# borgor/ripcurrents

Measured on AMD Instinct MI355X. Metric: frames/sec dense Farneback flow @1080p, higher is better.
Workload: dtype f32

## Files before the change

ripcurrents_amd/csrc/flow_iter_kernels.hip:

```cpp

#include <cstdlib>

#include "rc_device.h"

#define RC_ITER_BATCH 3
#define RC_RR_D 3

#ifdef RC_EXACT_BUILD
#define RC_FLOW_NS rc_flow_exact
#else
#define RC_FLOW_NS rc_flow_fast
#endif
namespace RC_FLOW_NS {

__device__ __forceinline__ float2 rc_flow_in(const RcIterArgs& a, const float2* fin, int gx, int gy) {
    if (a.in_mode == 0) return make_float2(0.f, 0.f);
    if (a.in_mode == 1) return fin[(size_t)gy * a.w + gx];
    float ax, ay;
    int sx = rc_src_x(gx, a.up_scale_x, a.fin_w, ax);
    int sx1 = min(sx + 1, a.fin_w - 1);
    int sy = rc_src_y(gy, a.up_scale_y, ay);
    int sy0 = rc_clampi(sy, 0, a.fin_h - 1), sy1 = rc_clampi(sy + 1, 0, a.fin_h - 1);
    const float2* S0 = fin + (size_t)sy0 * a.fin_w;
    const float2* S1 = fin + (size_t)sy1 * a.fin_w;
// ... 447 lines not shown
    for (int idx = tid; idx < 5 * CH * (TW / 4); idx += NT) {
        const int g4 = idx % (TW / 4), row = (idx / (TW / 4)) % CH, c = idx / (CH * (TW / 4));
        const float4* vp = (const float4*)(V + c * CH * VP + row * VP + 4 * g4);
        float v[4 * NQ];
#pragma unroll
        for (int q = 0; q < NQ; q++) {
            float4 t = vp[q];
            v[4 * q] = t.x; v[4 * q + 1] = t.y; v[4 * q + 2] = t.z; v[4 * q + 3] = t.w;
        }
        float o[4];
#pragma unroll
        for (int p = 0; p < 4; p++) {
            float s = v[M_ + p] * a.win.k[0];
#pragma unroll
            for (int i = 1; i <= M_; i++) s += a.win.k[i] * (v[M_ + p - i] + v[M_ + p + i]);
            o[p] = s;
        }
        *(float4*)(G + c * RING * MP + row * TW + 4 * g4) = make_float4(o[0], o[1], o[2], o[3]);
    }
    __syncthreads();
    for (int px = tid; px < CH * TW; px += NT) {
        const int row = px / TW, lx = px - row * TW;
        const int gx = tx0 + lx, gy = Y + row;
        double g[5];
#pragma unroll
        for (int c = 0; c < 5; c++) g[c] = G[c * RING * MP + px];
        if (gx < a.w && gy < yend) *(float2*)(fout + (size_t)gy * a.fout_step + (size_t)gx * 8) = rc_solve(g);
    }
    __syncthreads();
}

template <int M_, int NT, int BATCH>
__global__ __launch_bounds__(NT) void k_flow_iter_sweep(RcIterArgs a) {
    using S = RcSweep<M_>;
    constexpr int CH = S::CH, MW = S::MW, MP = S::MP, RING = S::RING, TW = S::TW;
    extern __shared__ __align__(16) float smf[];
    float* ring = smf;
    float* V = smf + 5 * RING * MP;
    const int tid = threadIdx.x;
    const int z = blockIdx.y;
    const int strip = blockIdx.x % a.tiles_x, seg = blockIdx.x / a.tiles_x;
    const int tx0 = strip * TW, y0 = seg * a.th;
    const int w = a.w, h = a.h;
    const int yend = min(y0 + a.th, h);
    const size_t s0 = (size_t)((a.slot0 + z * a.zstep) % a.nslots) * a.R_slot_stride;
    const size_t s1 = (size_t)((a.slot1 + z * a.zstep) % a.nslots) * a.R_slot_stride;
    const float4* RA0 = a.RA + s0;  const float* RB0 = a.RB + s0;
    const float4* RA1 = a.RA + s1;  const float* RB1 = a.RB + s1;
    const float2* fin = a.fin ? a.fin + (size_t)z * a.fin_pair_stride : nullptr;
    char* fout = a.fout + (size_t)z * a.fout_pair_stride;

    auto matrices_rows = [&](int r0, int nrows) {
        const int n = nrows * MW;
        for (int base = tid; base < n; base += NT * BATCH) {
            float2 d[BATCH];
            int gxs[BATCH], gys[BATCH];
#pragma unroll
            for (int q = 0; q < BATCH; q++) {
                const int idx = min(base + q * NT, n - 1);
                const int j = idx / MW, lx = idx - j * MW;
                gxs[q] = rc_clampi(tx0 - M_ + lx, 0, w - 1);
                gys[q] = rc_clampi(r0 + j, 0, h - 1);
                d[q] = rc_flow_in(a, fin, gxs[q], gys[q]);
            }
            RcM5 v[BATCH];
#pragma unroll
            for (int q = 0; q < BATCH; q++)
                v[q] = rc_matrices(RA0, RB0, RA1, RB1, gxs[q], gys[q], w, h, d[q].x, d[q].y);
#pragma unroll
            for (int q = 0; q < BATCH; q++) {
                const int idx = base + q * NT;
                if (idx < n) {
                    const int j = idx / MW, lx = idx - j * MW;
                    const int slot = (r0 + j - (y0 - M_)) % RING;
                    float* mp = ring + slot * MP + lx;
                    mp[0] = v[q].m0;
                    mp[RING * MP] = v[q].m1;
                    mp[2 * RING * MP] = v[q].m2;
                    mp[3 * RING * MP] = v[q].m3;
                    mp[4 * RING * MP] = v[q].m4;
                }
            }
        }
    };
    matrices_rows(y0 - M_, 2 * M_);
    const int nsteps = (yend - y0 + CH - 1) / CH;
    for (int s = 0; s < nsteps; s++) {
        matrices_rows(y0 + M_ + CH * s, CH);
        __syncthreads();
        const int Y = y0 + CH * s;
        switch (s % (RING / CH)) {
            case 0: rc_sweep_bc<M_, NT, 0>(a, ring, V, tid, tx0, Y, yend, fout); break;
            case 1: rc_sweep_bc<M_, NT, CH>(a, ring, V, tid, tx0, Y, yend, fout); break;
            case 2: rc_sweep_bc<M_, NT, 2 * CH>(a, ring, V, tid, tx0, Y, yend, fout); break;
            default: if constexpr (RING / CH > 3) rc_sweep_bc<M_, NT, 3 * CH>(a, ring, V, tid, tx0, Y, yend, fout); break;
        }
    }
}

template <int M, int NT, int BATCH>
static void launch_iter_sweep(RcIterArgs a, int pairs, hipStream_t s) {
    using S = RcSweep<M>;
    static_assert(S::RING / S::CH <= 4, "step dispatch covers four ring phases");
    RC_ALLOW_LDS((k_flow_iter_sweep<M, NT, BATCH>), S::LDS);
    a.tw = S::TW;
    a.tiles_x = (a.w + S::TW - 1) / S::TW;
    const int want = 4 * 512;
    int segs = (want + a.tiles_x * pairs - 1) / (a.tiles_x * pairs);
    int rs = (a.h + segs - 1) / segs;
    rs = ((rs + S::CH - 1) / S::CH) * S::CH;
    if (rs < 32) rs = 32;
    a.th = rs;
    a.tiles_y = (a.h + rs - 1) / rs;
    hipLaunchKernelGGL((k_flow_iter_sweep<M, NT, BATCH>), dim3(a.tiles_x * a.tiles_y, pairs, 1), dim3(NT), S::LDS, s, a);
}

#define RC_W3_THREADS 512
template <int IN_MODE, int GAUSS_>
__global__ __launch_bounds__(RC_W3_THREADS) void k_flow_iter_w3(RcIterArgs a) {
    constexpr int TW = 64, TH = 16, MW = TW + 2, MH = TH + 2, MP = MW | 1;
    constexpr int NITEMS = MW * MH, NIT = (NITEMS + RC_W3_THREADS - 1) / RC_W3_THREADS;
    extern __shared__ __align__(16) float smf[];
    float* Ms = smf;
    const int tid = threadIdx.x;
    const int z = blockIdx.y;
    const int t = a.xcd_remap ? rc_xcd_remap(blockIdx.x, a.tiles_x * a.tiles_y) : (int)blockIdx.x;
    const int tx0 = (t % a.tiles_x) * TW, ty0 = (t / a.tiles_x) * TH;
    const int w = a.w, h = a.h;
    const size_t s0 = (size_t)((a.slot0 + z * a.zstep) % a.nslots) * a.R_slot_stride;
    const size_t s1 = (size_t)((a.slot1 + z * a.zstep) % a.nslots) * a.R_slot_stride;
    const float4* __restrict__ RA0 = a.RA + s0;  const float* __restrict__ RB0 = a.RB + s0;
    const float4* __restrict__ RA1 = a.RA + s1;  const float* __restrict__ RB1 = a.RB + s1;
    const float2* __restrict__ fin = a.fin + (size_t)z * a.fin_pair_stride;
    char* fout = a.fout + (size_t)z * a.fout_pair_stride;

    int gx[NIT], gy[NIT];
#pragma unroll
    for (int q = 0; q < NIT; q++) {
        int idx = min(tid + q * RC_W3_THREADS, NITEMS - 1);
        int ly = idx / MW, lx = idx - ly * MW;
        gx[q] = rc_clampi(tx0 - 1 + lx, 0, w - 1);
        gy[q] = rc_clampi(ty0 - 1 + ly, 0, h - 1);
    }
    float dx[NIT], dy[NIT];
    if constexpr (IN_MODE == 0) {
#pragma unroll
        for (int q = 0; q < NIT; q++) dx[q] = dy[q] = 0.f;
    } else if constexpr (IN_MODE == 1) {
        float2 d[NIT];
#pragma unroll
        for (int q = 0; q < NIT; q++) d[q] = fin[(size_t)gy[q] * w + gx[q]];
#pragma unroll
        for (int q = 0; q < NIT; q++) { dx[q] = d[q].x; dy[q] = d[q].y; }
    } else {
        float2 p00[NIT], p01[NIT], p10[NIT], p11[NIT];
        float ax[NIT], ay[NIT];
#pragma unroll
        for (int q = 0; q < NIT; q++) {
            int sx = rc_src_x(gx[q], a.up_scale_x, a.fin_w, ax[q]);
            int sx1 = min(sx + 1, a.fin_w - 1);
            int sy = rc_src_y(gy[q], a.up_scale_y, ay[q]);
            int sy0 = rc_clampi(sy, 0, a.fin_h - 1), sy1 = rc_clampi(sy + 1, 0, a.fin_h - 1);
            const float2* S0 = fin + (size_t)sy0 * a.fin_w;
            const float2* S1 = fin + (size_t)sy1 * a.fin_w;
            p00[q] = S0[sx]; p01[q] = S0[sx1]; p10[q] = S1[sx]; p11[q] = S1[sx1];
        }
#pragma unroll
        for (int q = 0; q < NIT; q++) {
            float a0 = 1.f - ax[q], a1 = ax[q], b0 = 1.f - ay[q], b1 = ay[q];
            float r0x = p00[q].x * a0 + p01[q].x * a1, r1x = p10[q].x * a0 + p11[q].x * a1;
            float r0y = p00[q].y * a0 + p01[q].y * a1, r1y = p10[q].y * a0 + p11[q].y * a1;
            dx[q] = (r0x * b0 + r1x * b1) * a.up_mul;
            dy[q] = (r0y * b0 + r1y * b1) * a.up_mul;
        }
    }
    float4 A0[NIT];
    float B0[NIT];
    RcGather gt[NIT];
#pragma unroll
    for (int q = 0; q < NIT; q++) {
        size_t p0 = (size_t)gy[q] * w + gx[q];
        A0[q] = RA0[p0];
        B0[q] = RB0[p0];
        rc_gather_issue(gt[q], RA1, RB1, gx[q], gy[q], dx[q], dy[q], w, h);
    }
#pragma unroll
    for (int q = 0; q < NIT; q++) {
        RcM5 v = rc_matrices_reg(A0[q], B0[q], gt[q], dx[q], dy[q], gx[q], gy[q], w, h);
        int idx = tid + q * RC_W3_THREADS;
        if (idx < NITEMS) {
            int ly = idx / MW, lx = idx - ly * MW;
            float* mp = Ms + ly * MP + lx;
            mp[0] = v.m0;
            mp[MH * MP] = v.m1;
            mp[2 * MH * MP] = v.m2;
            mp[3 * MH * MP] = v.m3;
            mp[4 * MH * MP] = v.m4;
        }
    }
    __syncthreads();

    constexpr int RPT = TH / (RC_W3_THREADS / TW);
    const int lx = tid % TW, r0 = (tid / TW) * RPT;
    const int ox = tx0 + lx;
    float g[RPT][5];
#pragma unroll
    for (int c = 0; c < 5; c++) {
        const float* mc = Ms + c * MH * MP + r0 * MP + lx;
        float col[3][RPT + 2];
#pragma unroll
        for (int j = 0; j < 3; j++)
#pragma unroll
            for (int r = 0; r < RPT + 2; r++) col[j][r] = mc[r * MP + j];
#pragma unroll
        for (int r = 0; r < RPT; r++) {
            float v[3];
#pragma unroll
            for (int j = 0; j < 3; j++) {
                if (GAUSS_) v[j] = col[j][r + 1] * a.win.k[0] + (col[j][r + 2] + col[j][r]) * a.win.k[1];
                else v[j] = col[j][r + 1] + (col[j][r + 2] + col[j][r]);
            }
            if (GAUSS_) g[r][c] = v[1] * a.win.k[0] + a.win.k[1] * (v[0] + v[2]);
            else g[r][c] = (v[1] + v[0]) + v[2];
        }
    }
    if (ox < w) {
#pragma unroll
        for (int r = 0; r < RPT; r++) {
            int oy = ty0 + r0 + r;
            if (oy < h)
                *(float2*)(fout + (size_t)oy * a.fout_step + (size_t)ox * 8) =
                    rc_solve3(g[r], GAUSS_ ? 1e-3f : (float)a.win.box_eps);
        }
    }
}

template <int IN_MODE, int G>
static void launch_w3(RcIterArgs a, int pairs, hipStream_t s) {
    a.tw = 64; a.th = 16;
    a.tiles_x = (a.w + 63) / 64; a.tiles_y = (a.h + 15) / 16;
    size_t lds = sizeof(float) * 5 * 18 * 67;
    hipLaunchKernelGGL((k_flow_iter_w3<IN_MODE, G>), dim3(a.tiles_x * a.tiles_y, pairs, 1), dim3(RC_W3_THREADS), lds, s, a);
}

template <int WW, int WH, int WP = WW>
__device__ __forceinline__ void rc_gather_window(RcGather& g, const float4* LA, const float* LB, int ox, int oy,
                                                 const float4* __restrict__ RA1, const float* __restrict__ RB1,
                                                 int gx, int gy, float dx, float dy, int w, int h) {
    float fx = gx + dx, fy = gy + dy;
    int x1 = (int)floorf(fx), y1 = (int)floorf(fy);
    g.fx = fx - x1;
    g.fy = fy - y1;
    g.inside = (unsigned)x1 < (unsigned)(w - 1) && (unsigned)y1 < (unsigned)(h - 1);
    const int wx = x1 - ox, wy = y1 - oy;
    if (g.inside && (unsigned)wx < (unsigned)(WW - 1) && (unsigned)wy < (unsigned)(WH - 1)) {
        const int i = wy * WP + wx;
        g.q00 = LA[i]; g.q01 = LA[i + 1]; g.q10 = LA[i + WP]; g.q11 = LA[i + WP + 1];
        g.e00 = LB[i]; g.e01 = LB[i + 1]; g.e10 = LB[i + WP]; g.e11 = LB[i + WP + 1];
    } else {
        const size_t p = g.inside ? (size_t)y1 * w + x1 : (size_t)gy * w + gx;
        const size_t pw = g.inside ? (size_t)w : 0, p1 = g.inside ? 1 : 0;
        g.q00 = RA1[p]; g.q01 = RA1[p + p1]; g.q10 = RA1[p + pw]; g.q11 = RA1[p + pw + p1];
        g.e00 = RB1[p]; g.e01 = RB1[p + p1]; g.e10 = RB1[p + pw]; g.e11 = RB1[p + pw + p1];
    }
}

__device__ __forceinline__ void rc_hsum3_dpp(float (&g)[5], const float (&V)[5]) {
    float t0, t1, t2, t3, t4;
    asm("s_nop 1\n\t"
        "v_add_f32_dpp %5, %10, %10 wave_shr:1 row_mask:0xf bank_mask:0xf bound_ctrl:1\n\t"
        "v_add_f32_dpp %6, %11, %11 wave_shr:1 row_mask:0xf bank_mask:0xf bound_ctrl:1\n\t"
        "v_add_f32_dpp %7, %12, %12 wave_shr:1 row_mask:0xf bank_mask:0xf bound_ctrl:1\n\t"
        "v_add_f32_dpp %8, %13, %13 wave_shr:1 row_mask:0xf bank_mask:0xf bound_ctrl:1\n\t"
        "v_add_f32_dpp %9, %14, %14 wave_shr:1 row_mask:0xf bank_mask:0xf bound_ctrl:1\n\t"
        "v_add_f32_dpp %0, %10, %5 wave_shl:1 row_mask:0xf bank_mask:0xf bound_ctrl:1\n\t"
        "v_add_f32_dpp %1, %11, %6 wave_shl:1 row_mask:0xf bank_mask:0xf bound_ctrl:1\n\t"
        "v_add_f32_dpp %2, %12, %7 wave_shl:1 row_mask:0xf bank_mask:0xf bound_ctrl:1\n\t"
        "v_add_f32_dpp %3, %13, %8 wave_shl:1 row_mask:0xf bank_mask:0xf bound_ctrl:1\n\t"
        "v_add_f32_dpp %4, %14, %9 wave_shl:1 row_mask:0xf bank_mask:0xf bound_ctrl:1"
        : "=&v"(g[0]), "=&v"(g[1]), "=&v"(g[2]), "=&v"(g[3]), "=&v"(g[4]),
          "=&v"(t0), "=&v"(t1), "=&v"(t2), "=&v"(t3), "=&v"(t4)
        : "v"(V[0]), "v"(V[1]), "v"(V[2]), "v"(V[3]), "v"(V[4]));
}


__device__ __forceinline__ void rc_hpair_dpp(float (&s)[5], const float (&V)[5]) {
    float t0, t1, t2, t3, t4;
    asm("s_nop 1\n\t"
        "v_mov_b32_dpp %5, %10 wave_shr:1 row_mask:0xf bank_mask:0xf bound_ctrl:1\n\t"
        "v_mov_b32_dpp %6, %11 wave_shr:1 row_mask:0xf bank_mask:0xf bound_ctrl:1\n\t"
        "v_mov_b32_dpp %7, %12 wave_shr:1 row_mask:0xf bank_mask:0xf bound_ctrl:1\n\t"
        "v_mov_b32_dpp %8, %13 wave_shr:1 row_mask:0xf bank_mask:0xf bound_ctrl:1\n\t"
        "v_mov_b32_dpp %9, %14 wave_shr:1 row_mask:0xf bank_mask:0xf bound_ctrl:1\n\t"
        "v_add_f32_dpp %0, %10, %5 wave_shl:1 row_mask:0xf bank_mask:0xf bound_ctrl:1\n\t"
        "v_add_f32_dpp %1, %11, %6 wave_shl:1 row_mask:0xf bank_mask:0xf bound_ctrl:1\n\t"
        "v_add_f32_dpp %2, %12, %7 wave_shl:1 row_mask:0xf bank_mask:0xf bound_ctrl:1\n\t"
        "v_add_f32_dpp %3, %13, %8 wave_shl:1 row_mask:0xf bank_mask:0xf bound_ctrl:1\n\t"
        "v_add_f32_dpp %4, %14, %9 wave_shl:1 row_mask:0xf bank_mask:0xf bound_ctrl:1"
        : "=&v"(s[0]), "=&v"(s[1]), "=&v"(s[2]), "=&v"(s[3]), "=&v"(s[4]),
          "=&v"(t0), "=&v"(t1), "=&v"(t2), "=&v"(t3), "=&v"(t4)
        : "v"(V[0]), "v"(V[1]), "v"(V[2]), "v"(V[3]), "v"(V[4]));
}

template <int GAUSS_, int NIT, int MW, int NG>
__device__ __forceinline__ void rc_rr_flows(const float (&m)[NIT][5], const float* XR, int grp, int x,
                                            const RcWindow& win, float2 (&f)[NIT]) {
    const int gu = max(grp - 1, 0), gd = min(grp + 1, NG - 1);
    const int bu = (int)__umul24((unsigned)gu, 10u * MW) + x, bd = (int)__umul24((unsigned)gd, 10u * MW) + x;
    float up[5], dn[5];
#pragma unroll
    for (int c = 0; c < 5; c++) {
        up[c] = XR[bu + (5 + c) * MW];
        dn[c] = XR[bd + c * MW];
    }
    float V[NIT][5];
#pragma unroll
    for (int q = 0; q < NIT; q++)
#pragma unroll
        for (int c = 0; c < 5; c++) {
            float u = q > 0 ? m[q - 1][c] : up[c], d = q < NIT - 1 ? m[q + 1][c] : dn[c];
            if (GAUSS_) V[q][c] = m[q][c] * win.k[0] + (d + u) * win.k[1];
            else V[q][c] = m[q][c] + (d + u);
        }
#pragma unroll
    for (int q = 0; q < NIT; q++) {
        float g[5];
        if (GAUSS_) {
            float lr[5];
            rc_hpair_dpp(lr, V[q]);
#pragma unroll
            for (int c = 0; c < 5; c++) g[c] = V[q][c] * win.k[0] + win.k[1] * lr[c];
        } else {
            rc_hsum3_dpp(g, V[q]);
        }
        f[q] = rc_solve3(g, GAUSS_ ? 1e-3f : (float)win.box_eps);
    }
}

template <int NIT, int MW>
__device__ __forceinline__ void rc_rr_exchange(const float (&m)[NIT][5], float* XR, int grp, int x) {
    const int b = (int)__umul24((unsigned)grp, 10u * MW) + x;
#pragma unroll
    for (int c = 0; c < 5; c++) {
        XR[b + c * MW] = m[0][c];
        XR[b + (5 + c) * MW] = m[NIT - 1][c];
    }
}

template <int IN_MODE, int NIT, int MW, int MH, bool INTERIOR = false>
__device__ __forceinline__ void rc_rr_flow_in(const RcIterArgs& a, const float2* __restrict__ fin, int tx0, int ty0,
                                              int gxo, const int (&gys)[NIT], float (&dx)[NIT], float (&dy)[NIT]) {
    const int w = a.w, h = a.h;
    if constexpr (IN_MODE == 0) {
#pragma unroll
        for (int q = 0; q < NIT; q++) dx[q] = dy[q] = 0.f;
    } else if constexpr (IN_MODE == 1) {
        float2 d[NIT];
#pragma unroll
        for (int q = 0; q < NIT; q++) d[q] = INTERIOR ? fin[(unsigned)(gys[q] * w + gxo)] : fin[(size_t)gys[q] * w + gxo];
#pragma unroll
        for (int q = 0; q < NIT; q++) { dx[q] = d[q].x; dy[q] = d[q].y; }
    } else if ((NIT % 2 == 0) && a.up_exact2 && (INTERIOR || (ty0 - 2 >= 0 && ty0 - 2 + MH <= h))) {
        constexpr int NR = NIT / 2 + 2;
        int sx = (gxo - 1) >> 1;
        float ax = (gxo & 1) ? 0.25f : 0.75f;
        if (!INTERIOR) {
            if (sx < 0) { ax = 0.f; sx = 0; }
            if (sx >= a.fin_w - 1) { ax = 0.f; sx = a.fin_w - 1; }
        }
        const int sx1 = min(sx + 1, a.fin_w - 1);
        const int rb = (gys[0] - 1) >> 1;
        float2 t0[NR], t1[NR];
        typedef float rc_f4a8 __attribute__((ext_vector_type(4), aligned(8)));
        const bool cols_plain = INTERIOR || (tx0 - 2 >= 1 && tx0 - 2 + MW <= w && ((tx0 - 2 + MW - 2) >> 1) + 1 <= a.fin_w - 1);
        if (INTERIOR) {
            unsigned co = (unsigned)(__mul24(rb, a.fin_w) + sx);
#pragma unroll
            for (int j = 0; j < NR; j++) {
                const rc_f4a8 v = *(const rc_f4a8*)(fin + co);
                t0[j] = make_float2(v.x, v.y); t1[j] = make_float2(v.z, v.w);
                co += (unsigned)a.fin_w;
            }
        } else if (cols_plain) {
#pragma unroll
            for (int j = 0; j < NR; j++) {
                const float2* S = fin + (size_t)rc_clampi(rb + j, 0, a.fin_h - 1) * a.fin_w;
                const rc_f4a8 v = *(const rc_f4a8*)(S + sx);
                t0[j] = make_float2(v.x, v.y); t1[j] = make_float2(v.z, v.w);
            }
        } else {
#pragma unroll
            for (int j = 0; j < NR; j++) {
                const float2* S = fin + (size_t)rc_clampi(rb + j, 0, a.fin_h - 1) * a.fin_w;
                t0[j] = S[sx]; t1[j] = S[sx1];
            }
        }
        const float a0 = 1.f - ax, a1 = ax;
        float hx[NR], hy[NR];
#pragma unroll
        for (int j = 0; j < NR; j++) {
            hx[j] = t0[j].x * a0 + t1[j].x * a1;
            hy[j] = t0[j].y * a0 + t1[j].y * a1;
        }
#pragma unroll
        for (int q = 0; q < NIT; q++) {
            const int j0 = (q + 1) >> 1;
            const float b1 = (q & 1) ? 0.25f : 0.75f, b0 = 1.f - b1;
            dx[q] = (hx[j0] * b0 + hx[j0 + 1] * b1) * a.up_mul;
            dy[q] = (hy[j0] * b0 + hy[j0 + 1] * b1) * a.up_mul;
        }
    } else {
        float2 p00[NIT], p01[NIT], p10[NIT], p11[NIT];
        float ax, ay[NIT];
        int sx, sys[NIT];
        if (a.up_exact2) {
            sx = (gxo - 1) >> 1;
            ax = (gxo & 1) ? 0.25f : 0.75f;
            if (sx < 0) { ax = 0.f; sx = 0; }
            if (sx >= a.fin_w - 1) { ax = 0.f; sx = a.fin_w - 1; }
#pragma unroll
            for (int q = 0; q < NIT; q++) { sys[q] = (gys[q] - 1) >> 1; ay[q] = (gys[q] & 1) ? 0.25f : 0.75f; }
        } else {
            sx = rc_src_x(gxo, a.up_scale_x, a.fin_w, ax);
#pragma unroll
            for (int q = 0; q < NIT; q++) sys[q] = rc_src_y(gys[q], a.up_scale_y, ay[q]);
        }
        const int sx1 = min(sx + 1, a.fin_w - 1);
#pragma unroll
        for (int q = 0; q < NIT; q++) {
            int sy = sys[q];
            int sy0 = rc_clampi(sy, 0, a.fin_h - 1), sy1 = rc_clampi(sy + 1, 0, a.fin_h - 1);
            const float2* S0 = fin + (size_t)sy0 * a.fin_w;
            const float2* S1 = fin + (size_t)sy1 * a.fin_w;
            p00[q] = S0[sx]; p01[q] = S0[sx1]; p10[q] = S1[sx]; p11[q] = S1[sx1];
        }
#pragma unroll
        for (int q = 0; q < NIT; q++) {
            float a0 = 1.f - ax, a1 = ax, b0 = 1.f - ay[q], b1 = ay[q];
            float r0x = p00[q].x * a0 + p01[q].x * a1, r1x = p10[q].x * a0 + p11[q].x * a1;
            float r0y = p00[q].y * a0 + p01[q].y * a1, r1y = p10[q].y * a0 + p11[q].y * a1;
            dx[q] = (r0x * b0 + r1x * b1) * a.up_mul;
            dy[q] = (r0y * b0 + r1y * b1) * a.up_mul;
        }
    }
}


__device__ __forceinline__ void rc_lds_barrier() { asm volatile("s_waitcnt lgkmcnt(0)\n\ts_barrier" ::: "memory"); }
__device__ __forceinline__ void rc_all_barrier() { asm volatile("s_waitcnt vmcnt(0) lgkmcnt(0)\n\ts_barrier" ::: "memory"); }

constexpr bool rc_recip_exact(int nt, int wp) {
    const unsigned r = (65536u + wp - 1) / wp;
    for (int t = 0; t < nt; t++)
        if ((int)((t * r) >> 16) != t / wp) return false;
    return true;
}

__device__ __forceinline__ void rc_glds16_s(const void* base, unsigned voff, uint32_t lds_wave_addr) {
    asm volatile("s_mov_b32 m0, %2\n\ts_nop 0\n\tglobal_load_lds_dwordx4 %0, %1" ::"v"(voff), "s"(base), "s"(lds_wave_addr) : "memory");
}
__device__ __forceinline__ void rc_glds4_s(const void* base, unsigned voff, uint32_t lds_wave_addr) {
    asm volatile("s_mov_b32 m0, %2\n\ts_nop 0\n\tglobal_load_lds_dword %0, %1" ::"v"(voff), "s"(base), "s"(lds_wave_addr) : "memory");
}

template <bool INTERIOR, int NT, int WP, int WN, int NWL>
__device__ __forceinline__ void rc_rrc_issue_window(const float4* __restrict__ RA1, const float* __restrict__ RB1,
                                                    uint32_t lds_a, uint32_t lds_b, int tid, int ox, int oy, int w, int h) {
    constexpr int QY = NT / WP, QX = NT % WP;
    const int wave_base = __builtin_amdgcn_readfirstlane(tid & ~63);
    static_assert(rc_recip_exact(NT, WP), "tid / WP by multiply and shift must be exact for every thread");
    int wy = (int)(__umul24((unsigned)tid, (65536u + WP - 1) / WP) >> 16), wx = tid - (int)__umul24((unsigned)wy, (unsigned)WP);
    int off = __mul24(oy + wy, w) + ox + wx;
#pragma unroll
    for (int q = 0; q < NWL; q++) {
        bool ok = (q + 1) * NT <= WN || tid + q * NT < WN;
        if (!INTERIOR) ok = ok && (unsigned)(ox + wx) < (unsigned)w && (unsigned)(oy + wy) < (unsigned)h;
        const unsigned p = ok ? (unsigned)off : 0u;
        if (q * NT + wave_base < WN) {
            rc_glds16_s(RA1, p << 4, lds_a + (uint32_t)(q * NT + wave_base) * 16u);
            rc_glds4_s(RB1, p << 2, lds_b + (uint32_t)(q * NT + wave_base) * 4u);
        }
        wx += QX; wy += QY; off += QY * w + QX;
        if (wx >= WP) { wx -= WP; wy += 1; off += w - WP; }
    }
}

template <bool INTERIOR, int NIT, int WW, int WH, int WP>
__device__ __forceinline__ void rc_rr_matrices(float (&m)[NIT][5], const float4 (&A0)[NIT], const float (&B0)[NIT],
                                               const float (&dx)[NIT], const float (&dy)[NIT], const float4* LA,
                                               const float* LB, int ox, int oy, const float4* __restrict__ RA1,
                                               const float* __restrict__ RB1, int gxo, const int (&gys)[NIT], int w, int h) {
    if constexpr (!INTERIOR) {
#pragma unroll
        for (int q = 0; q < NIT; q++) {
            RcGather g;
            rc_gather_window<WW, WH, WP>(g, LA, LB, ox, oy, RA1, RB1, gxo, gys[q], dx[q], dy[q], w, h);
            RcM5 v = rc_matrices_reg(A0[q], B0[q], g, dx[q], dy[q], gxo, gys[q], w, h, true);
            m[q][0] = v.m0; m[q][1] = v.m1; m[q][2] = v.m2; m[q][3] = v.m3; m[q][4] = v.m4;
        }
    } else {
        unsigned far = 0;
#pragma unroll
        for (int q = 0; q < NIT; q++) {
            RcGather g;
            const float fx = gxo + dx[q], fy = gys[q] + dy[q];
            const float flx = floorf(fx), fly = floorf(fy);
            const int x1 = (int)flx, y1 = (int)fly;
            g.fx = fx - flx;
            g.fy = fy - fly;
            g.inside = true;
            const int wx = x1 - ox, wy = y1 - oy;
            const bool in_win = (unsigned)wx < (unsigned)(WW - 1) && (unsigned)wy < (unsigned)(WH - 1);
            far |= in_win ? 0u : 1u << q;
            const unsigned i = in_win ? __umul24((unsigned)wy, (unsigned)WP) + (unsigned)wx : 0u;
            const float4* pa = (const float4*)((const char*)LA + (i << 4));
            const float* pb = (const float*)((const char*)LB + (i << 2));
            g.q00 = pa[0]; g.q01 = pa[1]; g.q10 = pa[WP]; g.q11 = pa[WP + 1];
            g.e00 = pb[0]; g.e01 = pb[1]; g.e10 = pb[WP]; g.e11 = pb[WP + 1];
            RcM5 v = rc_matrices_reg(A0[q], B0[q], g, dx[q], dy[q], gxo, gys[q], w, h, false);
            m[q][0] = v.m0; m[q][1] = v.m1; m[q][2] = v.m2; m[q][3] = v.m3; m[q][4] = v.m4;
        }
        if (__builtin_expect(far != 0, 0)) {
#pragma unroll
            for (int q = 0; q < NIT; q++) {
                if (far >> q & 1) {
                    RcGather g;
                    rc_gather_issue(g, RA1, RB1, gxo, gys[q], dx[q], dy[q], w, h);
                    RcM5 v = rc_matrices_reg(A0[q], B0[q], g, dx[q], dy[q], gxo, gys[q], w, h, false);
                    m[q][0] = v.m0; m[q][1] = v.m1; m[q][2] = v.m2; m[q][3] = v.m3; m[q][4] = v.m4;
                }
            }
        }
    }
}

template <bool INTERIOR, int IN_MODE, int GAUSS_, int NIT, int D, int MW, int NG>
__device__ __forceinline__ void rc_rrc_body(const RcIterArgs& a, const int zb, const int ze, float* smf, const uint32_t lds0, const int tx0, const int ty0) {
    constexpr int NT = NG * MW, MH = NG * NIT;
    constexpr int WW = MW + 2 * D, WH = MH + 2 * D, WP = WW, WN = WP * WH, NWL = (WN + NT - 1) / NT;
    constexpr int WNP = (WN + 63) & ~63;
    constexpr int MP = MW + 1, PLANE = MH * MP;
    static_assert(5 * PLANE <= 5 * WNP, "border-block M1 planes alias the R1 window");
    float4* LA = (float4*)smf;
    float* LB = smf + 4 * WNP;
    float* XR = LB + WNP;
    float* Ms = smf;
    const uint32_t lds_a = lds0, lds_b = lds0 + 16u * WNP;
    const int w = a.w, h = a.h;
    const int ox = tx0 - 2 - D, oy = ty0 - 2 - D;
#define RC_RRC_COORDS(tid_)                                                         \
    const int x = (tid_) & (MW - 1), grp = (tid_) / MW, ly0 = grp * NIT;            \
    const int px = tx0 - 2 + x;                                                     \
    const int gxo = INTERIOR ? px : rc_clampi(px, 0, w - 1);                        \
    int gys[NIT];                                                                   \
    _Pragma("unroll") for (int q = 0; q < NIT; q++)                                 \
        gys[q] = INTERIOR ? ty0 - 2 + ly0 + q : rc_clampi(ty0 - 2 + ly0 + q, 0, h - 1);

    float4 A0[NIT];
    float B0[NIT];
    float dx[NIT], dy[NIT];
    {
        const int tid = threadIdx.x;
        RC_RRC_COORDS(tid)
        const size_t s0 = (size_t)((a.slot0 + zb * a.zstep) % a.nslots) * a.R_slot_stride;
        const size_t s1 = (size_t)((a.slot1 + zb * a.zstep) % a.nslots) * a.R_slot_stride;
        rc_rrc_issue_window<INTERIOR, NT, WP, WN, NWL>(a.RA + s1, a.RB + s1, lds_a, lds_b, tid, ox, oy, w, h);
#pragma unroll
        for (int q = 0; q < NIT; q++) {
            const unsigned p0 = (unsigned)(gys[q] * w + gxo);
            A0[q] = (a.RA + s0)[p0];
            B0[q] = (a.RB + s0)[p0];
        }
        rc_rr_flow_in<IN_MODE, NIT, MW, MH, INTERIOR>(a, a.fin + (size_t)zb * a.fin_pair_stride, tx0, ty0, gxo, gys, dx, dy);
    }

    for (int z = zb; z < ze; z++) {
        const size_t s1 = (size_t)((a.slot1 + z * a.zstep) % a.nslots) * a.R_slot_stride;
        const float4* __restrict__ RA1 = a.RA + s1;
        const float* __restrict__ RB1 = a.RB + s1;
        const bool more = z + 1 < ze;
        int tid = threadIdx.x;
        asm volatile("" : "+v"(tid));
        RC_RRC_COORDS(tid)
        rc_all_barrier();

        float m[NIT][5];
        rc_rr_matrices<INTERIOR, NIT, WW, WH, WP>(m, A0, B0, dx, dy, LA, LB, ox, oy, RA1, RB1, gxo, gys, w, h);
        rc_rr_exchange<NIT, MW>(m, XR, grp, x);
        rc_lds_barrier();

        {
            float2 f1[NIT];
            rc_rr_flows<GAUSS_, NIT, MW, NG>(m, XR, grp, x, a.win, f1);
            float f1x[NIT], f1y[NIT];
#pragma unroll
            for (int q = 0; q < NIT; q++) { f1x[q] = f1[q].x; f1y[q] = f1[q].y; }
            rc_rr_matrices<INTERIOR, NIT, WW, WH, WP>(m, A0, B0, f1x, f1y, LA, LB, ox, oy, RA1, RB1, gxo, gys, w, h);
        }
        if (more) {
#pragma unroll
            for (int q = 0; q < NIT; q++) {
                const int i = (int)__umul24((unsigned)(gys[q] - oy), (unsigned)WP) + (gxo - ox);
                A0[q] = LA[i];
                B0[q] = LB[i];
            }
        }
        rc_lds_barrier();
        if constexpr (!INTERIOR) {
#pragma unroll
            for (int q = 0; q < NIT; q++)
#pragma unroll
                for (int c = 0; c < 5; c++) Ms[c * PLANE + (ly0 + q) * MP + x] = m[q][c];
            rc_lds_barrier();
#pragma unroll
            for (int q = 0; q < NIT; q++) {
                const int py = ty0 - 2 + ly0 + q;
                if ((unsigned)px >= (unsigned)w || (unsigned)py >= (unsigned)h) {
                    const int cx = gxo - (tx0 - 2), cy = gys[q] - (ty0 - 2);
#pragma unroll
                    for (int c = 0; c < 5; c++) m[q][c] = Ms[c * PLANE + cy * MP + cx];
                }
            }
        }
        rc_rr_exchange<NIT, MW>(m, XR, grp, x);
        rc_lds_barrier();

        if (more) {
            const size_t n1 = (size_t)((a.slot1 + (z + 1) * a.zstep) % a.nslots) * a.R_slot_stride;
            rc_rrc_issue_window<INTERIOR, NT, WP, WN, NWL>(a.RA + n1, a.RB + n1, lds_a, lds_b, tid, ox, oy, w, h);
        }

        {
            char* fout = a.fout + (size_t)z * a.fout_pair_stride;
            float2 f2[NIT];
            rc_rr_flows<GAUSS_, NIT, MW, NG>(m, XR, grp, x, a.win, f2);
            if (x >= 2 && x < MW - 2 && (INTERIOR || px < w)) {
                unsigned so = (unsigned)(ty0 - 2 + ly0) * (unsigned)a.fout_step + (unsigned)px * 8u;
#pragma unroll
                for (int q = 0; q < NIT; q++) {
                    const int ly = ly0 + q, py = ty0 - 2 + ly;
                    if (ly >= 2 && ly < MH - 2 && (INTERIOR || py < h)) *(float2*)(fout + so) = f2[q];
                    so += (unsigned)a.fout_step;
                }
            }
        }
        if (more) rc_rr_flow_in<IN_MODE, NIT, MW, MH, INTERIOR>(a, a.fin + (size_t)(z + 1) * a.fin_pair_stride, tx0, ty0, gxo, gys, dx, dy);
    }
#undef RC_RRC_COORDS
}

template <int IN_MODE, int GAUSS_, int NIT, int D, int MINB, int MW, int NG>
__global__ __launch_bounds__(NG * MW, MINB) void k_flow_iter2_rrc(RcIterArgs a, RcChainPlan cp) {
    constexpr int MH = NG * NIT, TW = MW - 4, TH = MH - 4;
    extern __shared__ __align__(16) float smf[];
    const int zb = cp.ngroups ? cp.start[blockIdx.y] : (int)blockIdx.y, ze = cp.ngroups ? cp.start[blockIdx.y + 1] : zb + 1;
    const int t = a.xcd_remap ? rc_xcd_remap(blockIdx.x, a.tiles_x * a.tiles_y) : (int)blockIdx.x;
    const int tx0 = (t % a.tiles_x) * TW, ty0 = (t / a.tiles_x) * TH;
    const bool interior = tx0 - 2 >= 5 && tx0 - 2 + MW <= a.w - 5 && ty0 - 2 >= 5 && ty0 - 2 + MH <= a.h - 5;
    const uint32_t lds0 = (uint32_t)(uintptr_t)(__attribute__((address_space(3))) void*)smf;
    if (interior) rc_rrc_body<true, IN_MODE, GAUSS_, NIT, D, MW, NG>(a, zb, ze, smf, lds0, tx0, ty0);
    else rc_rrc_body<false, IN_MODE, GAUSS_, NIT, D, MW, NG>(a, zb, ze, smf, lds0, tx0, ty0);
}

template <int IN_MODE, int G, int NIT, int D, int MINB, int MW = 32, int NG = 8>
static void launch_rrc_t(RcIterArgs a, const RcChainPlan& cp, int pairs, hipStream_t s) {
    constexpr int MH = NG * NIT, TW = MW - 4, TH = MH - 4;
    a.tw = TW; a.th = TH;
    a.tiles_x = (a.w + TW - 1) / TW; a.tiles_y = (a.h + TH - 1) / TH;
    constexpr int WN = (MW + 2 * D) * (MH + 2 * D), WNP = (WN + 63) & ~63;
    const size_t lds = sizeof(float) * (5 * WNP + NG * 2 * 5 * MW);
    RC_ALLOW_LDS((k_flow_iter2_rrc<IN_MODE, G, NIT, D, MINB, MW, NG>), lds);
    hipLaunchKernelGGL((k_flow_iter2_rrc<IN_MODE, G, NIT, D, MINB, MW, NG>), dim3(a.tiles_x * a.tiles_y, cp.ngroups ? cp.ngroups : pairs, 1), dim3(NG * MW), lds, s, a, cp);
}

static void rc_chain_plan(const RcIterArgs& a, int pairs, long long tiles, RcChainPlan& cp) {
    cp.ngroups = 0;
    const bool chainable = a.chain > 1 && pairs > 1 && (a.slot0 + a.zstep) % a.nslots == a.slot1 % a.nslots;
    if (!chainable) return;
    int chain = a.chain;
    if (!(a.ablate & RC_ABL_FORCE_CHAIN))
        while (chain > 1 && tiles * pairs / chain < (a.chain_min_blocks > 0 ? a.chain_min_blocks : 4096)) chain >>= 1;
    if (chain <= 1) return;
    int n = 0, z = 0;
    cp.start[0] = 0;
    while (z < pairs) {
        int left = pairs - z, c = left > chain ? chain : (left + 1) / 2;
        if (n == RC_MAX_CHAIN_GROUPS - 1) c = left;
        z += c;
        cp.start[++n] = z;
    }
    cp.ngroups = n;
}

template <int IN_MODE, int G>
static void launch_w3x2(RcIterArgs a, int pairs, hipStream_t s) {
    const long long tiles = (long long)((a.w + 27) / 28) * ((a.h + 27) / 28), blocks = tiles * pairs;
    RcChainPlan cp;
    rc_chain_plan(a, pairs, tiles, cp);
    if (cp.ngroups) launch_rrc_t<IN_MODE, G, 4, RC_RR_D, 4>(a, cp, pairs, s);
    else if (blocks < 512) launch_rrc_t<IN_MODE, G, 2, 4, 6>(a, cp, pairs, s);
    else if (blocks < 1024) launch_rrc_t<IN_MODE, G, 3, 4, 5>(a, cp, pairs, s);
    else launch_rrc_t<IN_MODE, G, 4, RC_RR_D, 4>(a, cp, pairs, s);
}

int rc_flow_iter_can_fuse2(const RcIterArgs& a) { return a.win.m == 1 && a.solve && a.addr32; }

int rc_flow_iter2_r0_reads(const RcIterArgs& a, int pairs) {
    RcChainPlan cp;
    rc_chain_plan(a, pairs, (long long)((a.w + 27) / 28) * ((a.h + 27) / 28), cp);
    return cp.ngroups ? cp.ngroups : pairs;
}

int rc_flow_chain_groups(const RcIterArgs& a, int pairs, int* starts, int cap) {
    RcChainPlan cp;
    rc_chain_plan(a, pairs, (long long)((a.w + 27) / 28) * ((a.h + 27) / 28), cp);
    for (int i = 0; i <= cp.ngroups && i < cap; i++) starts[i] = cp.start[i];
    return cp.ngroups;
}

void rc_launch_flow_iter2(const RcIterArgs& a, int pairs, hipStream_t s) {
    const int g = a.win.gaussian ? 1 : 0;
    switch (a.in_mode * 2 + g) {
        case 0: launch_w3x2<0, 0>(a, pairs, s); break;
        case 1: launch_w3x2<0, 1>(a, pairs, s); break;
        case 2: launch_w3x2<1, 0>(a, pairs, s); break;
        case 3: launch_w3x2<1, 1>(a, pairs, s); break;
        case 4: launch_w3x2<2, 0>(a, pairs, s); break;
        default: launch_w3x2<2, 1>(a, pairs, s); break;
    }
}

static size_t iter_lds(int tw, int th, int m, bool two_buffers) {
    int MW = tw + 2 * m, MH = th + 2 * m, MP = MW | 1;
    return sizeof(float) * (5 * (size_t)MH * MP + (two_buffers ? 5 * (size_t)th * MP : 0));
}

template <int TW, int TH, int M, int G>
static void launch_iter_t(RcIterArgs a, int pairs, hipStream_t s) {
    size_t lds = iter_lds(TW, TH, M, M > 1);
    RC_ALLOW_LDS((k_flow_iter<TW, TH, M, G>), lds);
    a.tw = TW; a.th = TH;
    a.tiles_x = (a.w + TW - 1) / TW; a.tiles_y = (a.h + TH - 1) / TH;
    hipLaunchKernelGGL((k_flow_iter<TW, TH, M, G>), dim3(a.tiles_x * a.tiles_y, pairs, 1), dim3(RC_BLOCK), lds, s, a);
}

static void pick_runtime_tile(int m, int& tw, int& th) {
    static const int tiles[][2] = {{64, 16}, {32, 32}, {64, 8}, {32, 16}, {16, 16}, {16, 8}, {8, 8}};
    double best = -1;
    tw = 8; th = 8;
    for (auto& t : tiles) {
        size_t lds = iter_lds(t[0], t[1], m, true);
        if (lds > 150 * 1024) continue;
        double eff = (double)(t[0] * t[1]) / ((t[0] + 2 * m) * (t[1] + 2 * m));
        if (lds > 64 * 1024) eff *= 0.6;
        if (t[0] < 64) eff *= 0.95;
        if (eff > best) { best = eff; tw = t[0]; th = t[1]; }
    }
}

void rc_launch_flow_iter(const RcIterArgs& a, int pairs, hipStream_t s) {
    const int m = a.win.m, g = a.win.gaussian ? 1 : 0;
    if (m == 1 && a.solve) {
        switch (a.in_mode * 2 + g) {
            case 0: launch_w3<0, 0>(a, pairs, s); break;
            case 1: launch_w3<0, 1>(a, pairs, s); break;
            case 2: launch_w3<1, 0>(a, pairs, s); break;
            case 3: launch_w3<1, 1>(a, pairs, s); break;
            case 4: launch_w3<2, 0>(a, pairs, s); break;
            default: launch_w3<2, 1>(a, pairs, s); break;
        }
        return;
    }
    if (m == 1) { g ? launch_iter_t<64, 16, 1, 1>(a, pairs, s) : launch_iter_t<64, 16, 1, 0>(a, pairs, s); return; }
    if (a.solve) {
        if (m == 2) { g ? launch_iter_big<2, 1, 512>(a, pairs, s) : launch_iter_big<2, 0, 512>(a, pairs, s); return; }
        const long long work = (long long)a.w * a.h * pairs;
        if (g && (m == 5 || m == 10) && !(a.ablate & RC_ABL_TILE_WINDOW) &&
            ((a.ablate & RC_ABL_FORCE_SWEEP) || work >= (m == 10 ? 900000ll : 8000000ll))) {
            m == 5 ? launch_iter_sweep<5, 1024, 1>(a, pairs, s) : launch_iter_sweep<10, 1024, 1>(a, pairs, s);
            return;
        }
        if (m == 5) { g ? launch_iter_big<5, 1, 1024>(a, pairs, s) : launch_iter_big<5, 0, 1024>(a, pairs, s); return; }
        if (m == 10) { g ? launch_iter_big<10, 1, 1024, 64>(a, pairs, s) : launch_iter_big<10, 0, 1024, 64>(a, pairs, s); return; }
    }
    if (m == 2) { g ? launch_iter_t<64, 16, 2, 1>(a, pairs, s) : launch_iter_t<64, 16, 2, 0>(a, pairs, s); return; }
    if (m == 5) { g ? launch_iter_t<32, 32, 5, 1>(a, pairs, s) : launch_iter_t<32, 32, 5, 0>(a, pairs, s); return; }
    if (m == 10) { g ? launch_iter_t<32, 32, 10, 1>(a, pairs, s) : launch_iter_t<32, 32, 10, 0>(a, pairs, s); return; }
    RcIterArgs b = a;
    pick_runtime_tile(m, b.tw, b.th);
    b.tiles_x = (b.w + b.tw - 1) / b.tw; b.tiles_y = (b.h + b.th - 1) / b.th;
    size_t lds = iter_lds(b.tw, b.th, m, true);
    RC_ALLOW_LDS((k_flow_iter<0, 0, 0, 0>), lds);
    hipLaunchKernelGGL((k_flow_iter<0, 0, 0, 0>), dim3(b.tiles_x * b.tiles_y, pairs, 1), dim3(RC_BLOCK), lds, s, b);
}

}
```

ripcurrents_amd/csrc/rc_common.h:

```cpp
#pragma once

#include <hip/hip_runtime.h>
#include <limits.h>
#include <stdint.h>

#include "../../include/rcflow.h"
#include "rc_plan.h"

#define RC_FMA(a, b, c) __builtin_fmaf((a), (b), (c))

__device__ __forceinline__ int rc_cvt_i32_x86(float v) {
    return (v >= -2147483648.f && v < 2147483648.f) ? (int)v : (int)0x80000000;
}

__device__ __forceinline__ const float2* rc_row2(const float* base, size_t step, int y) {
    return (const float2*)((const char*)base + (size_t)y * step);
}

__device__ __forceinline__ bool rc_sample_flow(const float* flow, size_t step, int w, int h, float x, float y,
                                               float& dx, float& dy) {
    int xind = rc_cvt_i32_x86(floorf(x)), yind = rc_cvt_i32_x86(floorf(y));
    float xrem = x - xind, yrem = y - yind;
    if (xind < 1 || yind < 1 || xind + 2 > w || yind + 2 > h) return false;
    const float2* r0 = rc_row2(flow, step, yind) + xind;
    const float2* r1 = rc_row2(flow, step, yind + 1) + xind;
    float2 p00 = r0[0], p01 = r0[1], p10 = r1[0], p11 = r1[1];
    float wa = 1 - xrem, wb = 1 - yrem;
    dx = p00.x * wa * wb + p01.x * xrem * wb + p10.x * wa * yrem + p11.x * xrem * yrem;
    dy = p00.y * wa * wb + p01.y * xrem * wb + p10.y * wa * yrem + p11.y * xrem * yrem;
    return true;
}

__device__ __forceinline__ uint8_t rc_f2u8(float v) {
    int iv;
    if (!(v > -2147483904.f && v < 2147483648.f)) iv = INT_MIN;
    else iv = (int)v;
    return (uint8_t)(iv & 0xFF);
}

struct RcPyrArgs {
    const uint8_t* src;
    size_t src_step;
    size_t src_frame_stride;
    int W0, H0;
    float* dst;
    size_t dst_slot_stride;
    int dslot0, nslots, zstep;
    int w, h;
    double scale_x, scale_y;
    int ksize;
    const float* kern;
    int tw, th, reg_wp, reg_hmax;
    int direct;
    int fixed3;
};

struct RcPyrFused {
    float* dst;
    size_t dst_slot_stride;
    int w, h;
    const float* kern;
};

struct RcPolyArgs {
    const float* I;
    size_t I_slot_stride;
    const uint8_t* src8;
    size_t src8_step, src8_frame_stride;
    float4* RA;
    float* RB;
    size_t R_slot_stride;
    int slot0, nslots, zstep;
    int w, h;
    int tile_h;
    int valu_vertical;
    RcPolyK pk;
    int npyr;
    RcPyrFused py[2];
};

enum RcAblate : int {
    RC_ABL_EXACT_PLAIN_SCANS = 2,
    RC_ABL_EXACT_FUSED_M = 16,
    RC_ABL_PYR_STAGED = 4096,
    RC_ABL_TILE_WINDOW = 65536,
    RC_ABL_FORCE_SWEEP = 8388608,
    RC_ABL_FORCE_CHAIN = 33554432,
};

struct RcIterArgs {
    const float4* RA;
    const float* RB;
    size_t R_slot_stride;
    int slot0, slot1, nslots, zstep;
    int w, h;
    int in_mode;
    const float2* fin;
    size_t fin_pair_stride;
    int fin_w, fin_h;
    double up_scale_x, up_scale_y;
    float up_mul;
    int up_exact2;
    char* fout;
    size_t fout_step;
    size_t fout_pair_stride;
    int tw, th;
    int tiles_x, tiles_y;
    int solve;
    int xcd_remap;
    int ablate;
    int addr32;
    int chain_min_blocks;
    int chain;
    RcWindow win;
};

#define RC_MAX_CHAIN_GROUPS 64
struct RcChainPlan {
    int ngroups;
    int start[RC_MAX_CHAIN_GROUPS + 1];
};

struct RcExactArgs {
    const float4* RA;
    const float* RB;
    size_t n;
    int slot0, slot1, nslots, zstep;
    int w, h;
    const float2* fin;
    size_t fin_pair_stride;
    int fin_w, fin_h;
    double up_scale_x, up_scale_y;
    float up_mul;
    float2* flow;
    float* M;
    void* V;
    void* G;
    char* out;
    size_t out_step, out_pair_stride;
    int plain_scans;
    int fused_matrices;
    RcWindow win;
};
void rc_launch_exact_polyexp(const RcPolyArgs& a, int frames, hipStream_t s);
void rc_launch_exact_flow_init(const RcExactArgs& a, int pairs, hipStream_t s);
void rc_launch_exact_matrices(const RcExactArgs& a, int pairs, hipStream_t s);
void rc_launch_exact_window_solve(const RcExactArgs& a, int pairs, hipStream_t s);
int rc_exact_iteration_fused_ok(const RcExactArgs& a);
void rc_launch_exact_iteration_fused(const RcExactArgs& a, int pairs, hipStream_t s);

#define RC_MAX_DEVICES 64
#define RC_ALLOW_LDS(fn, lds)                                                                             \
    do {                                                                                                  \
        static size_t rc_seen_[RC_MAX_DEVICES] = {0};                                                     \
        int rc_dev_ = 0;                                                                                  \
        (void)hipGetDevice(&rc_dev_);                                                                     \
        if (rc_dev_ >= 0 && rc_dev_ < RC_MAX_DEVICES && (size_t)(lds) > rc_seen_[rc_dev_]) {             \
            (void)hipFuncSetAttribute((const void*)(fn), hipFuncAttributeMaxDynamicSharedMemorySize, (int)(lds)); \
            rc_seen_[rc_dev_] = (size_t)(lds);                                                            \
        }                                                                                                 \
    } while (0)

void rc_launch_pyr(const RcPyrArgs& a, int frames, size_t lds, hipStream_t s);
void rc_launch_polyexp(const RcPolyArgs& a, int frames, hipStream_t s);
int rc_polyexp_pyr_ok(const RcPolyArgs& a);
int rc_pyr_pair_ok(const RcPyrArgs& a1, const RcPyrArgs& a2);
void rc_launch_pyr_pair(const RcPyrArgs& a1, const RcPyrArgs& a2, int frames, hipStream_t s);
int rc_polyexp_multi_ok(const RcPolyArgs* a, int nlev);
void rc_launch_polyexp_multi(const RcPolyArgs* a, int nlev, int frames, hipStream_t s);
#define RC_FLOW_DECLS                                                         \
    void rc_launch_flow_iter(const RcIterArgs& a, int pairs, hipStream_t s);  \
     \
    int rc_flow_iter_can_fuse2(const RcIterArgs& a);                          \
    int rc_flow_iter2_r0_reads(const RcIterArgs& a, int pairs);               \
    int rc_flow_chain_groups(const RcIterArgs& a, int pairs, int* starts, int cap); \
    void rc_launch_flow_iter2(const RcIterArgs& a, int pairs, hipStream_t s);
namespace rc_flow_fast { RC_FLOW_DECLS }
namespace rc_flow_exact { RC_FLOW_DECLS }

struct RcFlowAreaArgs {
    const char* src;
    size_t src_step;
    size_t src_pair_stride;
    int W, H;
    float2* dst;
    size_t dst_pair_stride;
    int w, h;
    float mul;
    int fast, ix, iy;
    const int* xstart; const int* xsi; const float* xalpha;
    const int* ystart; const int* ysi; const float* yalpha;
    int lds_tab;
};
void rc_launch_flow_area_init(const RcFlowAreaArgs& a, int pairs, hipStream_t s);

void rc_launch_pack_R5(const float* R5, float4* RA, float* RB, int n, int fast_scale, hipStream_t s);
void rc_launch_unpack_R5(const float4* RA, const float* RB, float* R5, int n, int fast_scale, hipStream_t s);
```

ripcurrents_amd/csrc/rc_host.h:

```cpp
#pragma once

#include <initializer_list>
#include <string>
#include <vector>

#include "rc_args.h"
#include "rc_common.h"

struct RcBuf {
    void* p = nullptr;
    size_t bytes = 0;
};

struct RcPlan {
    bool valid = false;
    int w = 0, h = 0;
    rc_farneback_params prm{};
    int nlev = 0;
    RcLevel lv[RC_MAX_LEVELS];
    size_t kern_off[RC_MAX_LEVELS];
    RcPolyK pk;
    RcWindow win;
    int nslots = 0, chunk = 0;
    int exact_taps = 0;
// ... 9 lines not shown
    RcBuf thr;
    RcBuf acc;
    RcBuf pt;
    RcBuf dist;
    RcBuf scratch;
    RcBuf jet;
    RcBuf loopc;
};

struct RcLkPyr {
    int top; bool deriv;
    int lw[8], lh[8];
    size_t offI[8], offD[8], bytes;
};

struct RcZeroFence {
    hipEvent_t ev = nullptr;
    hipStream_t stream = nullptr;
    bool pending = false;
};

struct RcTimex {
    bool open = false;
    int w = 0, h = 0, window = 0, products = 0;
    int pitch = 0;
    size_t plane = 0;
    int cur = 0;
    long long frames = 0;
    RcBuf sum;
    RcBuf ring;
    RcBuf avg;
    RcBuf bd_idx[2], bd_hsv[2];
    RcZeroFence zf;
};

struct RcFrameStab {
    bool open = false;
    int w = 0, h = 0;
    int rx = 0, ry = 0, rw = 0, rh = 0;
    int N = 0, M = 0;
    size_t lds = 0;
    long long frames = 0;
    RcBuf tab;
    RcBuf prev;
    RcBuf res;
    RcBuf scratch;
    RcZeroFence zf;
    int n = 0, model = 0, flags = 0;
    double min_response = 0.;
    int px[RC_STAB_MAX_PATCHES] = {}, py[RC_STAB_MAX_PATCHES] = {};
    bool tracks = false;
    rc_stab_tracks tp{};
    int ncells = 0, margin = 0;
    RcLkPyr ref{}, cur{};
    RcBuf lkref, lkcur;
    RcBuf trk;
    int pcur = 0; bool pflip = false;
};
enum { RC_FT_RESULT = 0 , RC_FT_FIT = 4 , RC_FT_WS = 16 , RC_FT_DOUBLES = 18 };
enum { RC_FS_RESULT = 0 , RC_FS_MOTION = 3 , RC_FS_USED = 9 ,
       RC_FS_TICKET = 10 , RC_FS_SHIFTS = 16  };

struct RcRipMap {
    bool open = false;
    int w = 0, h = 0, window = 0, gx = 0, gy = 0, source = 0, flags = 0;
    int pitch = 0;
    int cur = 0;
    long long frames = 0;
    double K = 0.3454915028125263;
    double M = 0.;
    RcBuf ring;
    RcBuf avg;
    RcBuf acc;
    RcBuf out;
    RcZeroFence zf;
};

struct RcTrLineH { int kind, cap, n0; long long t_add; };
struct RcTracers {
    bool open = false;
    int w = 0, h = 0;
    rc_tracers_params prm{};
    std::vector<RcTrLineH> lines;
    int reserved = 0;
    int init_n = 0;
    int cur = 0;
    long long t = 0, t_reset = 0;
    long long dropped = 0;
    bool primed = false; int pyr_cur = 0;
    int nprims = 0;
    RcLkPyr plan{};
    RcBuf pyr;
    RcBuf pos;
    RcBuf init;
    RcBuf tab;
    RcBuf prims;
    RcBuf status;
    RcBuf ctr;
    RcZeroFence zf;
};

struct RcRegions {
    bool open = false;
    int w = 0, h = 0;
    rc_regions_params prm{};
    long long pushes = 0;
    RcBuf par;
    RcBuf area;
    RcBuf rows;
    RcBuf acc;
    RcBuf out;
    RcZeroFence zf;
};

struct RcTracks {
    bool open = false;
    int w = 0, h = 0;
    rc_tracks_params prm{};
    long long pushes = 0;
    RcBuf foot;
    RcBuf ov;
    RcBuf aux;
    RcBuf out;
    RcZeroFence zf;
};

struct RcMotion {
    bool open = false;
    int w = 0, h = 0;
    rc_motion_params prm{};
    int pitch = 0;
    long long pushes = 0;
    double last_ts = 0.;
    RcBuf mhi;
    RcBuf prev;
    RcBuf orient;
    RcBuf mask;
    RcBuf tab;
    RcBuf out;
    RcZeroFence zf;
};

struct RcFtle {
    bool open = false;
    int w = 0, h = 0;
    rc_ftle_params prm{};
    int pitch = 0;
    int cur = 0;
    long long pushes = 0;
    RcBuf ring;
    RcBuf map;
    RcBuf steps;
    RcBuf lam;
    RcBuf ctl;
    RcBuf out;
    RcBuf jet;
    RcZeroFence zf;
};

struct RcPlanView {
    bool open = false;
    int w = 0, h = 0;
    rc_planview_params prm{};
    long long pushes = 0;
    RcBuf table;
    RcBuf ctl;
    RcBuf out;
    RcZeroFence zf;
};

struct RcWaves {
    bool open = false;
    int w = 0, h = 0;
    rc_waves_params prm{};
    int K = 0;
    int pitch = 0;
    int sh = 0;
    long long pushes = 0;
    std::vector<int> tc, ts;
    RcBuf ring;
    RcBuf acc;
    RcBuf cacc;
    RcBuf out;
    RcBuf jet;
    RcZeroFence zf;
};

struct RcPiv {
    bool open = false;
    int w = 0, h = 0;
    rc_piv_params prm{};
    int gx = 0, gy = 0;
    int nw = 0;
    int pitch = 0;
    long long pushes = 0;
    RcBuf prev;
    RcBuf ring;
    RcBuf acc;
    RcBuf out;
    RcBuf ctl;
    RcBuf jet;
    RcZeroFence zf;
};

struct RcTransects {
    bool open = false;
    int w = 0, h = 0;
    rc_transects_params prm{};
    int L = 0, S = 0;
    int nw = 0;
    long long pushes = 0;
    RcBuf table;
    RcBuf ring_g;
    RcBuf ring_f;
    RcBuf acc;
    RcBuf out;
    RcBuf ctl;
    RcBuf jet;
    RcZeroFence zf;
};

struct RcKinematics {
    bool open = false;
    int w = 0, h = 0;
    rc_kinematics_params prm{};
    float taps[RC_KINEMATICS_MAX_RADIUS + 1] = {};
    long long pushes = 0;
    RcBuf planes;
    RcBuf acc;
    RcBuf out;
    RcBuf ctl;
    RcBuf jet;
    RcZeroFence zf;
};

struct RcShoreline {
    bool open = false;
    int w = 0, h = 0;
    rc_shoreline_params prm{};
    int L = 0, S = 0;
    long long pushes = 0;
    RcBuf table;
    RcBuf plane;
    RcBuf ring;
    RcBuf lin;
    RcBuf out;
    RcBuf ctl;
    RcZeroFence zf;
};

struct RcSurf {
    bool open = false;
    int w = 0, h = 0;
    rc_surf_params prm{};
    int L = 0, S = 0;
    int P = 0, tiles = 0;
    long long pushes = 0;
    RcBuf table;
    RcBuf ring;
    RcBuf bits;
    RcBuf sums;
    RcBuf out;
    RcBuf ctl;
    RcBuf jet;
    RcZeroFence zf;
};

struct RcWarpArgs {
    const uint8_t* src; size_t step;
    uint8_t* dst; size_t dst_step;
    int sw, sh, dw, dh;
    double M[9];
    const double* d_M;
    int bw0;
    float* patch;
    int npatch, rw, rh;
    int rx[RC_STAB_MAX_PATCHES], ry[RC_STAB_MAX_PATCHES];
};

struct RcPhaseCorr {
    int w = 0, h = 0;
    RcBuf tab, scratch;
};

struct RcGraphCache {
    void* exec[2] = {nullptr, nullptr};
    int eager[2] = {0, 0};
    unsigned char key[2][160] = {};
};

struct RcSlot {
    hipStream_t own = nullptr, cur = nullptr;
    hipStream_t aux = nullptr;
    hipEvent_t fev[8] = {nullptr, nullptr, nullptr, nullptr, nullptr, nullptr, nullptr, nullptr};
    int fev_i = 0;
    hipEvent_t flow_done[2] = {nullptr, nullptr};
    int flow_done_i = 0;
    int ts_streak = 0;
    bool in_ts_push = false;
    RcPlan plan;
    RcBuf kern;
    RcBuf I[RC_MAX_LEVELS], RA[RC_MAX_LEVELS], RB[RC_MAX_LEVELS];
    RcBuf FA[RC_MAX_LEVELS], FB[RC_MAX_LEVELS];
    RcBuf stage_u8, stage_flow, stage_f32[4];
    RcBuf exM, exV, exG;
    void* pin[2] = {nullptr, nullptr};
    size_t pin_bytes = 0;
    hipEvent_t pin_free[2] = {nullptr, nullptr};
    int pin_i = 0;
    int pin_acq = -1, pin_w = 0, pin_h = 0;
    int flow_w = 0, flow_h = 0;
    int flow_fresh = 0;
    RcBuf lk;
    RcBuf fit_ws;
    RcBuf area_tab;
    RcBuf seed, seed_tab;
    int primed = 0, cur_slot = 0;
    int batch_primed = 0, batch_cur = 0;
    RcGraphCache batch_graph;
    RcGraphCache loop_graph;
    int loop_fc = 0;
    RcAnalysis an;
    RcTimex tx;
    RcFrameStab fs;
    RcRipMap rm;
    RcTracers tr;
    RcRegions rg;
    RcTracks tk;
    RcMotion mt;
    RcFtle ft;
    RcPlanView pv;
    RcWaves wv;
    RcPiv piv;
    RcTransects ts;
    RcKinematics kn;
    RcShoreline sh;
    RcSurf sf;
    RcPhaseCorr pc;
};

struct RcProfRec {
    int id;
    hipEvent_t e0, e1;
    double bytes;
    double model_bytes;
};

struct rc_ctx {
    int device = 0;
    int max_w = 0, max_h = 0, nstreams = 0;
    RcSlot* slots = nullptr;
    int chunk = 32;
    int exact_taps = 0;
    int exact = -1;
    int fuse_iters = 1;
    int chain_min_blocks = 0;
    int chain = 8;
    int xcd_remap = 1;
    int poly_tile_h = 32;
    int frame_overlap = 1;
    int merge_small = 1;
    int overlap = 0;
    int poly_mfma = 0;
    int hist_blocks = 0;
    int fuse_pyr = 1;
    int ablate = 0;
    void* comm = nullptr;
    int prof_on = 0;
    std::vector<RcProfRec> prof_pending;
    std::vector<hipEvent_t> ev_pool;
    std::vector<int> prof_launches;
    std::vector<double> prof_ms, prof_bytes, prof_model_bytes;
};

#define RC_BUCKET_TABLE(X) \
    X(RC_B_FARNEBACK, "farneback") X(RC_B_POLAR, "polar") X(RC_B_THRESHOLD, "threshold") X(RC_B_OVERLAY, "overlay") \
    X(RC_B_EROSION, "erosion") X(RC_B_CODEC, "codec") X(RC_B_STREAM, "stream")
#define RC_KIND_TABLE(X) \
    X(RC_K_PYR, "pyr_level", RC_B_FARNEBACK) \
    X(RC_K_POLY, "polyexp", RC_B_FARNEBACK) \
    X(RC_K_ITER, "flow_iter", RC_B_FARNEBACK) \
    X(RC_K_HIST, "polar_hist", RC_B_THRESHOLD) \
    X(RC_K_THRESH, "thresholds", RC_B_THRESHOLD) \
    X(RC_K_CLASSIFY, "classify_accumulate", RC_B_THRESHOLD) \
    X(RC_K_ADVECT_FIELD, "advect_field", RC_B_STREAM) \
    X(RC_K_ADVECT_POINTS, "advect_points", RC_B_STREAM) \
    X(RC_K_POSTOP, "flow_postop", RC_B_FARNEBACK) \
    X(RC_K_COLOR, "flow_color", RC_B_THRESHOLD) \
    X(RC_K_ITER2, "flow_iter_x2", RC_B_FARNEBACK) \
    X(RC_K_PREPROC, "frame_preproc", RC_B_FARNEBACK) \
    X(RC_K_EDGES, "create_edges", RC_B_EROSION) \
    X(RC_K_DISPLAY, "streamline_display", RC_B_STREAM) \
    X(RC_K_HSV2BGR, "hsv_to_bgr", RC_B_THRESHOLD) \
    X(RC_K_OVERLAY, "create_output", RC_B_OVERLAY) \
    X(RC_K_FLOW_SEED, "flow_area_init", RC_B_FARNEBACK) \
    X(RC_K_TIMEX, "timex", RC_B_OVERLAY)  \
    X(RC_K_COLOR_U8, "frame_color", RC_B_OVERLAY)  \
    X(RC_K_FRAMESTAB, "framestab", RC_B_FARNEBACK)  \
    X(RC_K_RIPMAP, "ripmap", RC_B_FARNEBACK)  \
    X(RC_K_TRACKSTAB, "trackstab", RC_B_FARNEBACK)  \
    X(RC_K_TRACERS, "tracers", RC_B_STREAM)  \
    X(RC_K_REGIONS, "regions", RC_B_THRESHOLD)  \
    X(RC_K_TRACKS, "tracks", RC_B_THRESHOLD)  \
    X(RC_K_MOTION, "motion", RC_B_FARNEBACK)  \
    X(RC_K_FTLE, "ftle", RC_B_STREAM)  \
    X(RC_K_PLANVIEW, "planview", RC_B_FARNEBACK)  \
    X(RC_K_WAVES, "waves", RC_B_OVERLAY)  \
    X(RC_K_PIV, "piv", RC_B_FARNEBACK)  \
    X(RC_K_TRANSECTS, "transects", RC_B_STREAM)  \
    X(RC_K_KINEMATICS, "kinematics", RC_B_FARNEBACK)  \
    X(RC_K_SHORELINE, "shoreline", RC_B_OVERLAY)  \
    X(RC_K_SURF, "surf", RC_B_OVERLAY)
#define RC_ROW_ID(id, ...) id,
enum { RC_BUCKET_TABLE(RC_ROW_ID) RC_B_BUCKETS };
enum { RC_KIND_TABLE(RC_ROW_ID) RC_K_KINDS };
enum { RC_K_LISTED = RC_K_MOTION };
static_assert(RC_K_LISTED == 25, "the rows before RC_K_MOTION keep their ids");
static_assert(RC_B_BUCKETS == RC_PROFILE_BUCKETS, "include/rcflow.h promises RC_PROFILE_BUCKETS buckets");

int rc_buf_ensure(RcBuf& b, size_t bytes);
void rc_buf_free(RcBuf& b);
RcSlot* rc_slot(rc_ctx* ctx, int stream);
void rc_graph_drop(RcGraphCache& g);
int rc_classify_accumulate(const char* who, rc_ctx* ctx, int stream, const float* d_flow, size_t flow_step, int w, int h, int framecount,
                           float MID, float LOWER, float* d_polar, size_t polar_step, float* d_wclass, size_t wc_step,
                           float* d_out, size_t out_step, uint8_t* d_mask, size_t mask_step);
int rc_loop_counter(rc_ctx* ctx, RcSlot& s, bool set, int value);
int rc_hist_book(const char* who, RcSlot& s, int w, int h, bool commit);
int rc_analysis_ensure(const char* who, rc_ctx* ctx, RcSlot& s, int w, int h);
void rc_area_tab(int ssize, int dsize, double scale, std::vector<int>& start, std::vector<int>& si, std::vector<float>& alpha);
int rc_fence_zero(RcZeroFence& z, hipStream_t cur, std::initializer_list<RcBuf*> bufs);
int rc_fence_wait(RcZeroFence& z, hipStream_t cur, bool consume);
void rc_fence_free(RcZeroFence& z);
int rc_img3_check(const char* who, const char* what, const uint8_t* p, size_t step, int w, int h);
int rc_img3_pair(const char* who, const char* in_name, const uint8_t* in, size_t in_step, int sw, int sh, const char* out_name,
                 const uint8_t* out, size_t out_step, int dw, int dh);
int rc_fits_context(const char* who, const rc_ctx* ctx, int w, int h);
RcLkPyr rc_lk_plan(int w, int h, int win_w, int win_h, int max_level, bool deriv);
void rc_lk_build(rc_ctx* ctx, hipStream_t cur, const RcLkPyr& q, unsigned char* base);
void rc_lk_track(rc_ctx* ctx, hipStream_t cur_stream, const RcLkPyr& ref, const unsigned char* ref_base, const unsigned char* cur_base,
                 const RcLkPyr& cur, const float* d_prev_pts, float* d_next_pts, int npts, uint8_t* d_status, float* d_err, int win_w, int win_h,
                 int max_count, double epsilon, int flags, double min_eig_threshold);
void rc_gray_launch(rc_ctx* ctx, hipStream_t cur, const uint8_t* d_bgr, size_t step, int w, int h, uint8_t* d_gray);
int rc_corner_check(const char* who, int w, int h, int cells_x, int cells_y, int margin, int min_score);
void rc_corner_launch(rc_ctx* ctx, hipStream_t cur, const uint8_t* d_gray, size_t step, int w, int h, int cells_x, int cells_y, int margin,
                      int min_score, float* d_pts, int* d_scores);
int rc_fit_check(const char* who, int n, int w, int h, const rc_fit_params* prm);
void rc_fit_launch(rc_ctx* ctx, hipStream_t cur, const float* d_p, const float* d_q, const uint8_t* d_status, const int* d_scores, int n, int w,
                   int h, const rc_fit_params& prm, rc_fit_result* d_result, uint8_t* d_inlier, int* d_samples, void* d_ws, double* d_res,
                   double* d_res2);
void rc_advect_points_launch(rc_ctx* ctx, hipStream_t cur, float* d_pts, int n, const float* d_flow, size_t flow_step, int w, int h, float dt,
                             int iterations, float UPPER, const float* thr, int variant, float* d_trace);
void rc_draw_launch(rc_ctx* ctx, hipStream_t cur, uint8_t* d_img, size_t step, int w, int h, int channels, const rc_draw_prim* d_prims,
                    int n, unsigned long long* d_skipped);
void rc_warp_launch(rc_ctx* ctx, hipStream_t cur, RcWarpArgs& a, bool perspective);
int rc_line_plan(const char* who, int w, int h, const rc_transect_line& l, int i, int first, double metres_per_pixel, double fps,
                 rc_transect_sample* table, rc_transect_geom* geom);
int rc_flow_area_prepare(RcBuf& tab, int W, int H, int w, int h, RcFlowAreaArgs& a);

struct RcProfScope {
    rc_ctx* ctx;
    hipStream_t s;
    hipEvent_t e0 = nullptr, e1 = nullptr;
    int id;
    double bytes, model_bytes;
    RcProfScope(rc_ctx* c, hipStream_t st, int kind, int level, double alg_bytes, double survey_bytes = -1.);
    ~RcProfScope();
};

#define RC_HIP(call)                                                                  \
    do {                                                                              \
        hipError_t e_ = (call);                                                       \
        if (e_ != hipSuccess) {                                                       \
            rc_set_error("%s failed: %s (%s:%d)", #call, hipGetErrorString(e_), __FILE__, __LINE__); \
            return RC_EHIP;                                                           \
        }                                                                             \
    } while (0)

void rc_state_free(RcTimex& t);
void rc_state_free(RcFrameStab& f);
void rc_state_free(RcRipMap& m);
void rc_state_free(RcTracers& t);
void rc_state_free(RcRegions& g);
void rc_state_free(RcTracks& g);
void rc_state_free(RcMotion& m);
void rc_state_free(RcFtle& f);
void rc_state_free(RcPlanView& v);
void rc_state_free(RcWaves& v);
void rc_state_free(RcPiv& v);
void rc_state_free(RcTransects& v);
void rc_state_free(RcKinematics& k);
void rc_state_free(RcShoreline& v);
void rc_state_free(RcSurf& v);
int rc_state_zero(RcSlot& s, RcTimex& t);
int rc_state_zero(RcSlot& s, RcFrameStab& f);
int rc_state_zero(RcSlot& s, RcRipMap& m);
int rc_state_zero(RcSlot& s, RcTracers& t);
int rc_state_zero(RcSlot& s, RcRegions& g);
int rc_state_zero(RcSlot& s, RcTracks& g);
int rc_state_zero(RcSlot& s, RcMotion& m);
int rc_state_zero(RcSlot& s, RcFtle& f);
int rc_state_zero(RcSlot& s, RcPlanView& v);
int rc_state_zero(RcSlot& s, RcWaves& v);
int rc_state_zero(RcSlot& s, RcPiv& v);
int rc_state_zero(RcSlot& s, RcTransects& v);
int rc_state_zero(RcSlot& s, RcKinematics& k);
int rc_state_zero(RcSlot& s, RcShoreline& v);
int rc_state_zero(RcSlot& s, RcSurf& v);

template <class T>
int rc_state_install(RcSlot& s, T& cur, T& fresh, int rc) {
    if (!rc && cur.open && hipStreamSynchronize(s.cur) != hipSuccess) {
        rc_set_error("hipStreamSynchronize failed before a re-open");
        rc = RC_EHIP;
    }
    if (rc) {
        (void)hipGetLastError();
        rc_state_free(fresh);
        return rc;
    }
    rc_state_free(cur);
    cur = fresh;
    cur.open = true;
    if ((rc = rc_state_zero(s, cur))) rc_state_free(cur);
    return rc;
}

template <class T>
int rc_state_get(rc_ctx* ctx, int stream, T RcSlot::*member, const char* who, RcSlot*& s, T*& st) {
    if (!(s = rc_slot(ctx, stream))) return RC_EINVAL;
    st = &(s->*member);
    if (st->open) return RC_OK;
    rc_set_error("%s: the product is not open on the slot (its open call comes first)", who);
    return RC_ESTATE;
}

template <class T>
int rc_state_reset(rc_ctx* ctx, int stream, T RcSlot::*member, const char* who) {
    RcSlot* s; T* st;
    if (int rc = rc_state_get(ctx, stream, member, who, s, st)) return rc;
    RC_HIP(hipSetDevice(ctx->device));
    return rc_state_zero(*s, *st);
}

template <class T>
int rc_state_close(rc_ctx* ctx, int stream, T RcSlot::*member) {
    RcSlot* s = rc_slot(ctx, stream);
    if (!s) return RC_EINVAL;
    if (!(s->*member).open) return RC_OK;
    RC_HIP(hipSetDevice(ctx->device));
    RC_HIP(hipStreamSynchronize(s->cur));
    rc_state_free(s->*member);
    return RC_OK;
}
```

ripcurrents_amd/csrc/rc_plan.cpp:

```cpp

#include <cfloat>
#include <cmath>
#include <cstring>
#include <vector>

#include "rc_plan.h"

static inline int cv_round(double v) { return (int)nearbyint(v); }

int rc_plan_crop_levels(int w, int h, double pyr_scale, int levels) {
    const int min_size = 32;
    int k;
    double scale = 1;
    for (k = 0; k < levels; k++) {
        scale *= pyr_scale;
        if (w * scale < min_size || h * scale < min_size) break;
    }
    return k;
}

void rc_plan_level_geom(int w, int h, double pyr_scale, int k, RcLevel& L) {
    double scale = 1;
    for (int i = 0; i < k; i++) scale *= pyr_scale;
    L.sigma = (1. / scale - 1) * 0.5;
    int smooth_sz = cv_round(L.sigma * 5) | 1;
    L.ksize = smooth_sz > 3 ? smooth_sz : 3;
    L.w = cv_round(w * scale);
    L.h = cv_round(h * scale);
    L.scale_x = 1. / ((double)L.w / w);
    L.scale_y = 1. / ((double)L.h / h);
}

double rc_plan_scale_pow(double pyr_scale, int L) {
    double scale = 1;
    for (int i = 0; i < L; i++) scale *= pyr_scale;
    return scale;
}

void rc_plan_gaussian_kernel(int n, double sigma, float* cf) {
    static const float tab1[] = {1.f};
    static const float tab3[] = {0.25f, 0.5f, 0.25f};
    static const float tab5[] = {0.0625f, 0.25f, 0.375f, 0.25f, 0.0625f};
    static const float tab7[] = {0.03125f, 0.109375f, 0.21875f, 0.28125f, 0.21875f, 0.109375f, 0.03125f};
    const float* fixed = nullptr;
    if (n % 2 == 1 && n <= 7 && sigma <= 0) fixed = n == 1 ? tab1 : n == 3 ? tab3 : n == 5 ? tab5 : tab7;
    double sx = sigma > 0 ? sigma : ((n - 1) * 0.5 - 1) * 0.3 + 0.8;
    double scale2x = -0.5 / (sx * sx), sum = 0;
    for (int i = 0; i < n; i++) {
        double x = i - (n - 1) * 0.5;
        double t = fixed ? (double)fixed[i] : exp(scale2x * x * x);
        cf[i] = (float)t;
        sum += cf[i];
    }
    sum = 1. / sum;
    for (int i = 0; i < n; i++) cf[i] = (float)(cf[i] * sum);
}

int rc_plan_prepare_poly(int n, double sigma, int exact_taps, RcPolyK& pk) {
    if (sigma < FLT_EPSILON) sigma = n * 0.3;
    std::vector<float> gb(2 * n + 1), xgb(2 * n + 1), xxgb(2 * n + 1);
    float *g = gb.data() + n, *xg = xgb.data() + n, *xxg = xxgb.data() + n;
    double s = 0.;
    for (int x = -n; x <= n; x++) {
        g[x] = (float)exp(-x * x / (2 * sigma * sigma));
        s += g[x];
    }
    s = 1. / s;
    for (int x = -n; x <= n; x++) {
        g[x] = (float)(g[x] * s);
        xg[x] = (float)(x * g[x]);
        xxg[x] = (float)(x * x * g[x]);
    }
    double G[6][6] = {{0}};
    for (int y = -n; y <= n; y++)
        for (int x = -n; x <= n; x++) {
            G[0][0] += g[y] * g[x];
            G[1][1] += g[y] * g[x] * x * x;
            G[3][3] += g[y] * g[x] * x * x * x * x;
            G[5][5] += g[y] * g[x] * x * x * y * y;
        }
    G[2][2] = G[0][3] = G[0][4] = G[3][0] = G[4][0] = G[1][1];
    G[4][4] = G[3][3];
    G[3][4] = G[4][3] = G[5][5];
    double L[6][6], inv[6][6];
    for (int i = 0; i < 6; i++)
        for (int j = 0; j < 6; j++) { L[i][j] = G[i][j]; inv[i][j] = i == j ? 1. : 0.; }
    for (int i = 0; i < 6; i++) {
        double v;
        int j, k;
        for (j = 0; j < i; j++) {
            v = L[i][j];
            for (k = 0; k < j; k++) v -= L[i][k] * L[j][k];
            L[i][j] = v * L[j][j];
        }
        v = L[i][i];
        for (k = 0; k < j; k++) { double t = L[i][k]; v -= t * t; }
        if (!(v >= DBL_EPSILON)) return RC_EINVAL;
        L[i][i] = 1. / sqrt(v);
    }
    for (int i = 0; i < 6; i++)
        for (int j = 0; j < 6; j++) {
            double v = inv[i][j];
            for (int k = 0; k < i; k++) v -= L[i][k] * inv[k][j];
            inv[i][j] = v * L[i][i];
        }
    for (int i = 5; i >= 0; i--)
        for (int j = 0; j < 6; j++) {
            double v = inv[i][j];
            for (int k = 5; k > i; k--) v -= L[k][i] * inv[k][j];
            inv[i][j] = v * L[i][i];
        }
    pk.ig11 = inv[1][1];
    pk.ig03 = inv[0][3];
    pk.ig33 = inv[3][3];
    pk.ig55 = inv[5][5];
    pk.n = n;
    int n_thr = n;
    if (!exact_taps) {
        double m0 = 0, m1 = 0, m2 = 0;
        for (int k = 1; k <= n; k++) { m0 += g[k]; m1 += fabs(xg[k]); m2 += xxg[k]; }
        double t0 = 0, t1 = 0, t2 = 0;
        for (int k = n; k >= 1; k--) {
            t0 += g[k]; t1 += fabs(xg[k]); t2 += xxg[k];
            if (t0 > 1e-8 * (m0 + g[0]) || t1 > 1e-8 * m1 || t2 > 1e-8 * m2) break;
            n_thr = k - 1;
        }
        if (n_thr < 1) n_thr = 1;
    }
    static const int inst[] = {3, 5, 7, 8, 9, 12, 16, 24, 32};
    int R = 32;
    for (int v : inst)
        if (v >= n_thr) { R = v; break; }
    pk.n_eff = R < n ? R : n;
    memset(pk.g, 0, sizeof(pk.g));
    memset(pk.xg, 0, sizeof(pk.xg));
    memset(pk.xxg, 0, sizeof(pk.xxg));
    double sg = 0, s2 = 0;
    for (int k = 0; k <= pk.n_eff; k++) {
        pk.g[k] = g[k];
        pk.xg[k] = xg[k];
        pk.xxg[k] = xxg[k];
        sg += (k ? 2. : 1.) * g[k];
        s2 += (k ? 2. : 0.) * xxg[k];
    }
    pk.kdc = sg * sg * pk.ig03 + sg * s2 * pk.ig33;
    memset(pk.qh, 0, sizeof(pk.qh));
    memset(pk.xga, 0, sizeof(pk.xga));
    memset(pk.xgb, 0, sizeof(pk.xgb));
    const double sa = pk.ig11 * 0.5, sb = (pk.ig55 * 0.25) / sa;
    for (int k = 0; k <= pk.n_eff; k++) {
        pk.qh[k] = (float)(0.5 * (pk.ig03 * (double)g[k] + pk.ig33 * (double)xxg[k]));
        pk.xga[k] = (float)((double)xg[k] * sa);
        pk.xgb[k] = (float)((double)xg[k] * sb);
    }
    pk.kdch = 0.5 * pk.kdc;
    return RC_OK;
}

void rc_plan_window(int winsize, int flags, RcWindow& win) {
    int m = winsize / 2;
    memset(&win, 0, sizeof(win));
    win.m = m;
    win.gaussian = (flags & RC_FARNEBACK_GAUSSIAN) ? 1 : 0;
    win.box_scale = 1. / ((double)winsize * winsize);
    win.box_eps = 1e-3 / (win.box_scale * win.box_scale);
    double sigma = m * 0.3, s = 1;
    win.k[0] = (float)s;
    for (int i = 1; i <= m; i++) {
        float t = (float)exp(-i * i / (2 * sigma * sigma));
        win.k[i] = t;
        s += t * 2;
    }
    s = 1. / s;
    for (int i = 0; i <= m; i++) win.k[i] = (float)(win.k[i] * s);
}

void rc_plan_pick_pyr_tile(RcLevel& L, int W0, int H0) {
    static const int tiles[][2] = {{64, 16}, {64, 8}, {64, 4}, {32, 8}, {16, 8}, {16, 4}, {8, 4}, {4, 4}, {2, 2}, {1, 1}};
    int r = L.ksize / 2;
    for (auto& t : tiles) {
        int tw = t[0], th = t[1];
        int rw = (int)ceil(tw * L.scale_x) + 2 * r + 4;
        int rh = (int)ceil(th * L.scale_y) + 2 * r + 4;
        if (rw > W0 + 2 * r + 2) rw = W0 + 2 * r + 2;
        if (rh > H0 + 2 * r + 2) rh = H0 + 2 * r + 2;
        int rwp = (rw + 15) & ~15;
        size_t lds = (size_t)rh * rwp + sizeof(float) * ((size_t)rh * 2 * tw + 3 * tw + 3 * th + L.ksize);
        if (lds <= 40 * 1024 || tw == 1) {
            L.pyr_tw = tw; L.pyr_th = th; L.pyr_reg_w = rwp; L.pyr_reg_h = rh; L.pyr_lds = lds;
            return;
        }
    }
}

int rc_plan_params_valid(const rc_farneback_params* p) {
    if (!p) return 0;
    if (!(p->pyr_scale > 0 && p->pyr_scale < 1)) return 0;
    if (p->levels < 0 || p->levels >= RC_MAX_LEVELS) return 0;
    if (p->winsize < 1 || p->winsize / 2 > 24) return 0;
    if (p->iterations < 0 || p->iterations > 1000) return 0;
    if (p->poly_n < 1 || p->poly_n > RC_MAX_POLY_N) return 0;
    if (!(p->poly_sigma >= 0)) return 0;
    if (p->flags & ~(RC_FARNEBACK_GAUSSIAN | RC_FARNEBACK_USE_INITIAL_FLOW)) return 0;
    return 1;
}
```

ripcurrents_amd/csrc/rc_plan.h:

```cpp
#pragma once

#include <stddef.h>

#include "../../include/rcflow.h"

#define RC_MAX_LEVELS 12
#define RC_MAX_POLY_N 32
#define RC_MAX_WIN_M 32

struct RcLevel {
    int w, h;
    double scale_x;
    double scale_y;
    double sigma;
    int ksize;
    int pyr_tw, pyr_th;
    int pyr_reg_w, pyr_reg_h;
    size_t pyr_lds;
};

struct RcPolyK {
    float g[RC_MAX_POLY_N + 1];
    float xg[RC_MAX_POLY_N + 1];
    float xxg[RC_MAX_POLY_N + 1];
    double ig11, ig03, ig33, ig55;
    double kdc;
    int n;
    int n_eff;
    float qh[RC_MAX_POLY_N + 1];
    float xga[RC_MAX_POLY_N + 1];
    float xgb[RC_MAX_POLY_N + 1];
    double kdch;
};

struct RcWindow {
    float k[RC_MAX_WIN_M + 1];
    double box_scale;
    double box_eps;
    int m;
    int gaussian;
};

int rc_plan_params_valid(const rc_farneback_params* p);
int rc_plan_crop_levels(int w, int h, double pyr_scale, int levels);
void rc_plan_level_geom(int w, int h, double pyr_scale, int k, RcLevel& L);
double rc_plan_scale_pow(double pyr_scale, int L);
void rc_plan_pick_pyr_tile(RcLevel& L, int W0, int H0);
void rc_plan_gaussian_kernel(int n, double sigma, float* cf);
int rc_plan_prepare_poly(int n, double sigma, int exact_taps, RcPolyK& pk);
void rc_plan_window(int winsize, int flags, RcWindow& win);
```

ripcurrents_amd/csrc/rcflow_api.hip:

```cpp

#include <cfloat>
#include <climits>
#include <cmath>
#include <cstdarg>
#include <cstdio>
#include <cstring>

#include "rc_host.h"

static thread_local char g_err[512] = "";
void rc_set_error(const char* fmt, ...) {
    va_list ap;
    va_start(ap, fmt);
    vsnprintf(g_err, sizeof(g_err), fmt, ap);
    va_end(ap);
}
extern "C" const char* rcflow_last_error(void) { return g_err; }
extern "C" int rcflow_abi_version(void) { return RCFLOW_ABI_VERSION; }

int rc_buf_ensure(RcBuf& b, size_t bytes) {
    if (b.bytes >= bytes && b.p) return RC_OK;
    if (b.p) (void)hipFree(b.p);
    b.p = nullptr;
    b.bytes = 0;
    if (bytes == 0) return RC_OK;
    hipError_t e = hipMalloc(&b.p, bytes);
    if (e != hipSuccess) {
        rc_set_error("hipMalloc(%zu) failed: %s", bytes, hipGetErrorString(e));
        b.p = nullptr;
        return RC_ENOMEM;
    }
    b.bytes = bytes;
    return RC_OK;
}
void rc_buf_free(RcBuf& b) {
    if (b.p) (void)hipFree(b.p);
    b.p = nullptr;
    b.bytes = 0;
}
RcSlot* rc_slot(rc_ctx* ctx, int stream) {
    if (!ctx || stream < 0 || stream >= ctx->nstreams) {
        rc_set_error("bad context or stream index %d", stream);
        return nullptr;
    }
    return &ctx->slots[stream];
}

int rc_fence_zero(RcZeroFence& z, hipStream_t cur, std::initializer_list<RcBuf*> bufs) {
    for (RcBuf* b : bufs)
        if (b->p) RC_HIP(hipMemsetAsync(b->p, 0, b->bytes, cur));
    if (!z.ev) RC_HIP(hipEventCreateWithFlags(&z.ev, hipEventDisableTiming));
    RC_HIP(hipEventRecord(z.ev, cur));
    z.stream = cur;
    z.pending = true;
    return RC_OK;
}
int rc_fence_wait(RcZeroFence& z, hipStream_t cur, bool consume) {
    if (!z.pending) return RC_OK;
    if (cur != z.stream) RC_HIP(hipStreamWaitEvent(cur, z.ev, 0));
    if (consume) z.pending = false;
    return RC_OK;
}
void rc_fence_free(RcZeroFence& z) {
    if (z.ev) (void)hipEventDestroy(z.ev);
    z = RcZeroFence();
}

int rc_img3_check(const char* who, const char* what, const uint8_t* p, size_t step, int w, int h) {
    return rc_image_check(who, what, p, step, w, h, 3, 1, RC_ARG_IN);
}
int rc_img3_pair(const char* who, const char* in_name, const uint8_t* in, size_t in_step, int sw, int sh, const char* out_name,
                 const uint8_t* out, size_t out_step, int dw, int dh) {
    RcArgs a(who, sw, sh);
    a.image(in_name, in, in_step, 3, 1, RC_ARG_IN);
    a.image(out_name, out, out_step, 3, 1, RC_ARG_OUT, dw, dh);
    return a.check();
}
int rc_fits_context(const char* who, const rc_ctx* ctx, int w, int h) {
    if (w <= ctx->max_w && h <= ctx->max_h) return RC_OK;
    rc_set_error("%s: %d x %d exceeds the context size %d x %d", who, w, h, ctx->max_w, ctx->max_h);
    return RC_ESIZE;
}

RcProfScope::RcProfScope(rc_ctx* c, hipStream_t st, int kind, int level, double alg_bytes, double survey_bytes)
    : ctx(c), s(st), id(kind * RC_MAX_LEVELS + level), bytes(alg_bytes),
      model_bytes(survey_bytes < 0 ? alg_bytes : survey_bytes) {
    if (!ctx->prof_on) return;
    for (int i = 0; i < 2; i++) {
        hipEvent_t e;
        if (!ctx->ev_pool.empty()) {
            e = ctx->ev_pool.back();
            ctx->ev_pool.pop_back();
        } else if (hipEventCreate(&e) != hipSuccess) {
            e = nullptr;
        }
        (i ? e1 : e0) = e;
    }
    if (e0) (void)hipEventRecord(e0, s);
}
RcProfScope::~RcProfScope() {
    if (!ctx->prof_on || !e0 || !e1) return;
    (void)hipEventRecord(e1, s);
    ctx->prof_pending.push_back({id, e0, e1, bytes, model_bytes});
}

#define RC_ROW_NAME(id, name, ...) name,
#define RC_ROW_BUCKET(id, name, bucket) bucket,
static const char* const kKindNames[RC_K_KINDS] = {RC_KIND_TABLE(RC_ROW_NAME)};
static const int kBucketOfKind[RC_K_KINDS] = {RC_KIND_TABLE(RC_ROW_BUCKET)};
static const char* const kBucketNames[RC_B_BUCKETS] = {RC_BUCKET_TABLE(RC_ROW_NAME)};
static char g_names[RC_K_KINDS * RC_MAX_LEVELS][40];

static void prof_resolve(rc_ctx* ctx) {
    size_t n = RC_K_KINDS * RC_MAX_LEVELS;
    if (ctx->prof_ms.size() != n) {
        ctx->prof_ms.assign(n, 0.);
        ctx->prof_bytes.assign(n, 0.);
        ctx->prof_model_bytes.assign(n, 0.);
        ctx->prof_launches.assign(n, 0);
    }
    for (auto& r : ctx->prof_pending) {
        float ms = 0.f;
        (void)hipEventSynchronize(r.e1);
        if (hipEventElapsedTime(&ms, r.e0, r.e1) == hipSuccess) {
            ctx->prof_ms[r.id] += ms;
            ctx->prof_bytes[r.id] += r.bytes;
            ctx->prof_model_bytes[r.id] += r.model_bytes;
            ctx->prof_launches[r.id]++;
        }
        ctx->ev_pool.push_back(r.e0);
        ctx->ev_pool.push_back(r.e1);
    }
    ctx->prof_pending.clear();
}

extern "C" int rcflow_profile_enable(rc_ctx* ctx, int on) {
    if (int rc = rc_ptr_check(__func__, "ctx", ctx)) return rc;
    if (!on) prof_resolve(ctx);
    ctx->prof_on = on ? 1 : 0;
    return RC_OK;
}
extern "C" int rcflow_profile_reset(rc_ctx* ctx) {
    if (int rc = rc_ptr_check(__func__, "ctx", ctx)) return rc;
    prof_resolve(ctx);
    ctx->prof_ms.assign(ctx->prof_ms.size(), 0.);
    ctx->prof_bytes.assign(ctx->prof_bytes.size(), 0.);
    ctx->prof_model_bytes.assign(ctx->prof_model_bytes.size(), 0.);
    ctx->prof_launches.assign(ctx->prof_launches.size(), 0);
    return RC_OK;
}
extern "C" int rcflow_profile_read(rc_ctx* ctx, int cap, const char** names, int* launches,
                                   double* total_ms, double* alg_bytes, double* model_bytes) {
    if (int rc = rc_ptr_check(__func__, "ctx", ctx)) return rc;
    prof_resolve(ctx);
    int n = 0;
    for (size_t id = 0; id < ctx->prof_ms.size() && n < cap; id++) {
        if (!ctx->prof_launches[id]) continue;
        snprintf(g_names[id], sizeof(g_names[id]), "%s@%d", kKindNames[id / RC_MAX_LEVELS],
                 (int)(id % RC_MAX_LEVELS));
        if (names) names[n] = g_names[id];
        if (launches) launches[n] = ctx->prof_launches[id];
        if (total_ms) total_ms[n] = ctx->prof_ms[id];
        if (alg_bytes) alg_bytes[n] = ctx->prof_bytes[id];
        if (model_bytes) model_bytes[n] = ctx->prof_model_bytes[id];
        n++;
    }
    return n;
}

extern "C" int rcflow_profile_read_buckets(rc_ctx* ctx, const char** names, double* ms) {
    if (int rc = rc_ptr_check(__func__, "ctx", ctx)) return rc;
    prof_resolve(ctx);
    double b[RC_PROFILE_BUCKETS] = {0};
    for (size_t id = 0; id < ctx->prof_ms.size(); id++) b[kBucketOfKind[id / RC_MAX_LEVELS]] += ctx->prof_ms[id];
    for (int i = 0; i < RC_PROFILE_BUCKETS; i++) {
        if (names) names[i] = kBucketNames[i];
        if (ms) ms[i] = b[i];
    }
    return RC_PROFILE_BUCKETS;
}

extern "C" int rcflow_create(rc_ctx** out, int device, int max_w, int max_h, int max_streams) {
    if (!out || max_w <= 0 || max_h <= 0 || max_streams <= 0 || max_streams > 256) {
        rc_set_error("rcflow_create: bad arguments");
        return RC_EINVAL;
    }
    *out = nullptr;
    int ndev = 0;
    if (hipGetDeviceCount(&ndev) != hipSuccess || ndev <= 0 || device < 0 || device >= ndev) {
        rc_set_error("rcflow_create: no usable HIP device (count=%d, requested %d)", ndev, device);
        return RC_ENODEV;
    }
    RC_HIP(hipSetDevice(device));
    hipDeviceProp_t prop;
    RC_HIP(hipGetDeviceProperties(&prop, device));
    if (strncmp(prop.gcnArchName, "gfx950", 6) != 0) {
        rc_set_error("rcflow_create: device %d is %s; this library holds gfx950 code only", device,
                     prop.gcnArchName);
        return RC_ENODEV;
    }
    rc_ctx* ctx = new rc_ctx();
    ctx->device = device;
    ctx->max_w = max_w;
    ctx->max_h = max_h;
    ctx->nstreams = max_streams;
    ctx->slots = new RcSlot[max_streams];
    for (int i = 0; i < max_streams; i++) {
        hipError_t e = hipStreamCreateWithFlags(&ctx->slots[i].own, hipStreamNonBlocking);
        if (e != hipSuccess) {
            rc_set_error("rcflow_create: hipStreamCreate failed: %s", hipGetErrorString(e));
            rcflow_destroy(ctx);
            return RC_EHIP;
        }
        ctx->slots[i].cur = ctx->slots[i].own;
    }
    *out = ctx;
    return RC_OK;
}

static void slot_free(RcSlot& s) {
    rc_buf_free(s.kern);
    for (int k = 0; k < RC_MAX_LEVELS; k++) {
        rc_buf_free(s.I[k]); rc_buf_free(s.RA[k]); rc_buf_free(s.RB[k]);
        rc_buf_free(s.FA[k]); rc_buf_free(s.FB[k]);
    }
    rc_graph_drop(s.batch_graph);
    rc_buf_free(s.stage_u8); rc_buf_free(s.stage_flow); rc_buf_free(s.lk); rc_buf_free(s.fit_ws); rc_buf_free(s.area_tab);
    rc_buf_free(s.seed); rc_buf_free(s.seed_tab);
    rc_buf_free(s.exM); rc_buf_free(s.exV); rc_buf_free(s.exG);
    for (int i = 0; i < 2; i++) {
        if (s.pin[i]) (void)hipHostFree(s.pin[i]);
        if (s.pin_free[i]) (void)hipEventDestroy(s.pin_free[i]);
        s.pin[i] = nullptr; s.pin_free[i] = nullptr;
    }
    s.pin_bytes = 0;
    for (auto& b : s.stage_f32) rc_buf_free(b);
    rc_buf_free(s.an.hist); rc_buf_free(s.an.hist_part); rc_buf_free(s.an.thr); rc_buf_free(s.an.acc);
    rc_buf_free(s.an.pt); rc_buf_free(s.an.dist); rc_buf_free(s.an.scratch); rc_buf_free(s.an.jet); rc_buf_free(s.an.loopc);
    rc_state_free(s.tx);
    rc_state_free(s.fs);
    rc_state_free(s.rm);
    rc_state_free(s.tr);
    rc_state_free(s.rg);
    rc_state_free(s.tk);
    rc_state_free(s.mt);
    rc_state_free(s.ft);
    rc_state_free(s.pv);
    rc_state_free(s.wv);
    rc_state_free(s.piv);
    rc_state_free(s.ts);
    rc_state_free(s.kn);
    rc_state_free(s.sh);
    rc_state_free(s.sf);
    rc_buf_free(s.pc.tab); rc_buf_free(s.pc.scratch);
    rc_graph_drop(s.loop_graph);
    for (auto& e : s.fev) { if (e) (void)hipEventDestroy(e); e = nullptr; }
    for (auto& e : s.flow_done) { if (e) (void)hipEventDestroy(e); e = nullptr; }
    if (s.own) (void)hipStreamDestroy(s.own);
    if (s.aux) (void)hipStreamDestroy(s.aux);
    s.aux = nullptr;
    s.own = s.cur = nullptr;
}

extern "C" void rcflow_destroy(rc_ctx* ctx) {
    if (!ctx) return;
    (void)hipSetDevice(ctx->device);
    (void)hipDeviceSynchronize();
    (void)rcflow_comm_destroy(ctx);
    prof_resolve(ctx);
    for (auto e : ctx->ev_pool) (void)hipEventDestroy(e);
    if (ctx->slots) {
        for (int i = 0; i < ctx->nstreams; i++) slot_free(ctx->slots[i]);
        delete[] ctx->slots;
    }
    delete ctx;
}

extern "C" int rcflow_sync(rc_ctx* ctx, int stream) {
    RcSlot* s = rc_slot(ctx, stream);
    if (!s) return RC_EINVAL;
    RC_HIP(hipStreamSynchronize(s->cur));
    return RC_OK;
}

extern "C" int rcflow_set_hip_stream(rc_ctx* ctx, int stream, void* hip_stream) {
    RcSlot* s = rc_slot(ctx, stream);
    if (!s) return RC_EINVAL;
    s->cur = (hipStream_t)hip_stream;
    return RC_OK;
}

extern "C" int rcflow_use_own_stream(rc_ctx* ctx, int stream) {
    RcSlot* s = rc_slot(ctx, stream);
    if (!s) return RC_EINVAL;
    s->cur = s->own;
    return RC_OK;
}

extern "C" int rcflow_debug_chain_plan(int w, int h, int pairs, int chain, int force, int* starts, int cap) {
    if (w <= 0 || h <= 0 || pairs < 1 || cap < 2) { rc_set_error("%s: w %d, h %d, pairs %d (>= 1) or cap %d (>= 2)", __func__, w, h, pairs, cap); return RC_EINVAL; }
    if (int rc = rc_ptr_check(__func__, "starts", starts)) return rc;
    RcIterArgs a;
    memset(&a, 0, sizeof(a));
    a.w = w; a.h = h; a.chain = chain; a.addr32 = 1; a.slot0 = 0; a.slot1 = 1; a.zstep = 1; a.nslots = pairs + 1;
    a.ablate = force ? RC_ABL_FORCE_CHAIN : 0;
    return rc_flow_fast::rc_flow_chain_groups(a, pairs, starts, cap);
}

extern "C" int rcflow_debug_level_flow_ptr(rc_ctx* ctx, int stream, int level, int which, float** d_flow, int* w, int* h) {
    RcSlot* s = rc_slot(ctx, stream);
    if (!s) return RC_EINVAL;
    if (!s->plan.valid || level < 0 || level >= s->plan.nlev) { rc_set_error("%s: no plan on the slot, or level %d outside it", __func__, level); return RC_EINVAL; }
    if (int rc = rc_ptr_check(__func__, "d_flow", d_flow)) return rc;
    *d_flow = (float*)(which ? s->FB[level].p : s->FA[level].p);
    if (w) *w = s->plan.lv[level].w;
    if (h) *h = s->plan.lv[level].h;
    if (*d_flow) return RC_OK;
    rc_set_error("%s: the level has no flow field yet", __func__);
    return RC_ESTATE;
}

static int poly_prepare(const char* who, int n, double sigma, int exact_taps, RcPolyK& pk) {
    const int rc = rc_plan_prepare_poly(n, sigma, exact_taps, pk);
    if (rc) rc_set_error("%s: polynomial-expansion moment matrix is not positive definite", who);
    return rc;
}

extern "C" int rcflow_debug_plan_poly(int n, double sigma, int exact_taps, float* g, float* xg, float* xxg, double* ig, int* n_eff,
                                      double* kdc) {
    if (n < 1 || n > RC_MAX_POLY_N || !(sigma >= 0)) { rc_set_error("%s: n %d (1..%d) or sigma %g (>= 0)", __func__, n, RC_MAX_POLY_N, sigma); return RC_EINVAL; }
    if (!g || !xg || !xxg || !ig || !n_eff || !kdc) { rc_set_error("%s: a null pointer among g, xg, xxg, ig, n_eff, kdc", __func__); return RC_EINVAL; }
    RcPolyK pk;
    if (int rc = poly_prepare(__func__, n, sigma, exact_taps, pk)) return rc;
    memcpy(g, pk.g, (n + 1) * sizeof(float));
    memcpy(xg, pk.xg, (n + 1) * sizeof(float));
    memcpy(xxg, pk.xxg, (n + 1) * sizeof(float));
    ig[0] = pk.ig11; ig[1] = pk.ig03; ig[2] = pk.ig33; ig[3] = pk.ig55;
    *n_eff = pk.n_eff;
    *kdc = pk.kdc;
    return RC_OK;
}
extern "C" int rcflow_debug_plan_poly_folded(int n, double sigma, int exact_taps, float* qh, float* xga, float* xgb, double* kdch) {
    if (n < 1 || n > RC_MAX_POLY_N || !(sigma >= 0)) { rc_set_error("%s: n %d (1..%d) or sigma %g (>= 0)", __func__, n, RC_MAX_POLY_N, sigma); return RC_EINVAL; }
    if (!qh || !xga || !xgb || !kdch) { rc_set_error("%s: a null pointer among qh, xga, xgb, kdch", __func__); return RC_EINVAL; }
    RcPolyK pk;
    if (int rc = poly_prepare(__func__, n, sigma, exact_taps, pk)) return rc;
    memcpy(qh, pk.qh, (n + 1) * sizeof(float));
    memcpy(xga, pk.xga, (n + 1) * sizeof(float));
    memcpy(xgb, pk.xgb, (n + 1) * sizeof(float));
    *kdch = pk.kdch;
    return RC_OK;
}
extern "C" int rcflow_debug_plan_pyr_kernel(int ksize, double sigma, float* taps) {
    if (ksize < 1 || ksize > 1023 || !(sigma >= 0)) { rc_set_error("%s: ksize %d (1..1023) or sigma %g (>= 0)", __func__, ksize, sigma); return RC_EINVAL; }
    if (int rc = rc_ptr_check(__func__, "taps", taps)) return rc;
    rc_plan_gaussian_kernel(ksize, sigma, taps);
    return RC_OK;
}
extern "C" int rcflow_debug_kind(int id, const char** name, const char** bucket) {
    if (id < 0 || id >= RC_K_LISTED) { rc_set_error("%s: id %d (0..%d)", __func__, id, RC_K_LISTED - 1); return RC_EINVAL; }
    if (!name || !bucket) { rc_set_error("%s: a null pointer among name, bucket", __func__); return RC_EINVAL; }
    *name = kKindNames[id];
    *bucket = kBucketNames[kBucketOfKind[id]];
    return RC_OK;
}

extern "C" int rcflow_set_option(rc_ctx* ctx, const char* name, int value) {
    const char* who = __func__;
    if (!ctx || !name) { rc_set_error("%s: a null pointer among ctx, name", who); return RC_EINVAL; }
    auto outside = [&](int lo, int hi) {
        if (value >= lo && value <= hi) return false;
        rc_set_error("%s: %s = %d is outside %d..%d", who, name, value, lo, hi);
        return true;
    };
    if (!strcmp(name, "chunk")) {
        if (outside(1, 64)) return RC_EINVAL;
        ctx->chunk = value;
    } else if (!strcmp(name, "exact_taps")) {
        ctx->exact_taps = value ? 1 : 0;
    } else if (!strcmp(name, "exact")) {
        if (outside(-1, 1)) return RC_EINVAL;
        ctx->exact = value;
    } else if (!strcmp(name, "fuse_iters")) {
        ctx->fuse_iters = value ? 1 : 0;
    } else if (!strcmp(name, "chain")) {
        if (outside(1, 64)) return RC_EINVAL;
        ctx->chain = value;
    } else if (!strcmp(name, "chain_min_blocks")) {
        if (outside(0, INT_MAX)) return RC_EINVAL;
        ctx->chain_min_blocks = value;
    } else if (!strcmp(name, "xcd_remap")) {
        ctx->xcd_remap = value ? 1 : 0;
    } else if (!strcmp(name, "hist_blocks")) {
        if (outside(0, 65535)) return RC_EINVAL;
        ctx->hist_blocks = value;
    } else if (!strcmp(name, "overlap")) {
        ctx->overlap = value ? 1 : 0;
    } else if (!strcmp(name, "frame_overlap")) {
        if (outside(0, 2)) return RC_EINVAL;
        ctx->frame_overlap = value;
    } else if (!strcmp(name, "merge_small")) {
        ctx->merge_small = value ? 1 : 0;
    } else if (!strcmp(name, "poly_mfma")) {
        ctx->poly_mfma = value ? 1 : 0;
    } else if (!strcmp(name, "poly_tile_h")) {
        if (value != 32 && value != 48) { rc_set_error("%s: poly_tile_h = %d is neither 32 nor 48", who, value); return RC_EINVAL; }
        ctx->poly_tile_h = value;
    } else if (!strcmp(name, "fuse_pyr")) {
        ctx->fuse_pyr = value != 0;
    } else if (!strcmp(name, "ablate")) {
        ctx->ablate = value;
    } else {
        rc_set_error("%s: unknown option %s", who, name);
        return RC_EINVAL;
    }
    for (int i = 0; i < ctx->nstreams; i++) ctx->slots[i].plan.valid = false;
    return RC_OK;
}

extern "C" int rcflow_level_geometry(int w, int h, double pyr_scale, int levels, int k, int* wk, int* hk) {
    if (w <= 0 || h <= 0 || !(pyr_scale > 0 && pyr_scale < 1) || levels < 0 || k < 0) {
        rc_set_error("%s: size %d x %d, pyr_scale %g (inside 0..1), levels %d or k %d (>= 0)", __func__, w, h, pyr_scale, levels, k);
        return RC_EINVAL;
    }
    RcLevel L;
    rc_plan_level_geom(w, h, pyr_scale, k, L);
    if (wk) *wk = L.w;
    if (hk) *hk = L.h;
    return rc_plan_crop_levels(w, h, pyr_scale, levels);
}

static int ensure_plan(const char* who, rc_ctx* ctx, RcSlot& s, int w, int h, const rc_farneback_params* p, int chunk, int nslots = 0) {
    if (nslots <= 0) nslots = chunk + 1;
    if (w <= 0 || h <= 0 || !rc_plan_params_valid(p)) {
        rc_set_error("%s: invalid Farneback arguments (w=%d h=%d)", who, w, h);
        return RC_EINVAL;
    }
    if (int rc = rc_fits_context(who, ctx, w, h)) return rc;
    RcPlan& pl = s.plan;
    const rc_farneback_params& q = pl.prm;
    const bool same_prm = q.pyr_scale == p->pyr_scale && q.levels == p->levels && q.winsize == p->winsize &&
                          q.iterations == p->iterations && q.poly_n == p->poly_n && q.poly_sigma == p->poly_sigma &&
                          q.flags == p->flags;
    const int exact = ctx->exact >= 0 ? ctx->exact
                                      : (p->winsize / 2 == 0 || ((p->flags & RC_FARNEBACK_GAUSSIAN) && p->winsize / 2 <= 2));
    if (pl.valid && pl.w == w && pl.h == h && same_prm && pl.chunk == chunk &&
        pl.nslots == nslots && pl.exact_taps == ctx->exact_taps && pl.exact == exact)
        return RC_OK;
    rc_graph_drop(s.batch_graph);
    rc_graph_drop(s.loop_graph);
    RC_HIP(hipStreamSynchronize(s.cur));
    if (s.aux) RC_HIP(hipStreamSynchronize(s.aux));
    pl.valid = false;
    pl.w = w; pl.h = h; pl.chunk = chunk; pl.nslots = nslots;
    memset(&pl.prm, 0, sizeof(pl.prm));
    pl.prm.pyr_scale = p->pyr_scale; pl.prm.levels = p->levels; pl.prm.winsize = p->winsize;
    pl.prm.iterations = p->iterations; pl.prm.poly_n = p->poly_n; pl.prm.poly_sigma = p->poly_sigma;
    pl.prm.flags = p->flags;
    pl.exact_taps = ctx->exact_taps;
    pl.exact = exact;
    int L = rc_plan_crop_levels(w, h, p->pyr_scale, p->levels);
    pl.nlev = L + 1;
    size_t kern_total = 0;
    for (int k = 0; k <= L; k++) {
        rc_plan_level_geom(w, h, p->pyr_scale, k, pl.lv[k]);
        if (pl.lv[k].ksize > 1023) { rc_set_error("%s: pyramid blur too wide", who); return RC_EINVAL; }
        rc_plan_pick_pyr_tile(pl.lv[k], w, h);
        pl.kern_off[k] = kern_total;
        kern_total += (pl.lv[k].ksize + 3) & ~3;
    }
    int rc = poly_prepare(who, p->poly_n, p->poly_sigma, ctx->exact_taps || exact, pl.pk);
    if (rc) return rc;
    rc_plan_window(p->winsize, p->flags, pl.win);

    std::vector<float> kh(kern_total, 0.f);
    for (int k = 0; k <= L; k++) rc_plan_gaussian_kernel(pl.lv[k].ksize, pl.lv[k].sigma > 0 ? pl.lv[k].sigma : 0., kh.data() + pl.kern_off[k]);
    if ((rc = rc_buf_ensure(s.kern, kern_total * sizeof(float)))) return rc;
    RC_HIP(hipMemcpy(s.kern.p, kh.data(), kern_total * sizeof(float), hipMemcpyHostToDevice));
    for (int k = 0; k <= L; k++) {
        size_t n = (size_t)pl.lv[k].w * pl.lv[k].h;
        if ((k > 0 || exact) && (rc = rc_buf_ensure(s.I[k], n * pl.nslots * sizeof(float)))) return rc;
        if ((rc = rc_buf_ensure(s.RA[k], n * pl.nslots * sizeof(float4)))) return rc;
        if ((rc = rc_buf_ensure(s.RB[k], n * pl.nslots * sizeof(float)))) return rc;
        if ((rc = rc_buf_ensure(s.FA[k], n * chunk * sizeof(float2)))) return rc;
        if ((rc = rc_buf_ensure(s.FB[k], n * chunk * sizeof(float2)))) return rc;
    }
    memset(&pl.seed, 0, sizeof(pl.seed));
    if (p->flags & RC_FARNEBACK_USE_INITIAL_FLOW) {
        if ((rc = rc_flow_area_prepare(s.seed_tab, w, h, pl.lv[L].w, pl.lv[L].h, pl.seed))) return rc;
        pl.seed.mul = (float)rc_plan_scale_pow(p->pyr_scale, L);
    }
    s.primed = 0;
    s.batch_primed = 0;
    pl.valid = true;
    return RC_OK;
}

struct RcSeed {
    const float* field;
    size_t step, pair_stride;
};

static int seed_layout_ok(const char* who, const void* p, size_t step, size_t pair_stride) {
    if ((((uintptr_t)p) | step | pair_stride) & 7) { rc_set_error("%s: initial flow: pointer and strides must be multiples of 8 bytes", who); return 0; }
    return 1;
}

static int launch_seed(rc_ctx* ctx, RcSlot& s, int pairs, const RcSeed& seed, const float2** out) {
    RcPlan& pl = s.plan;
    const int k = pl.nlev - 1;
    const size_t n = (size_t)pl.lv[k].w * pl.lv[k].h;
    int rc;
    if ((rc = rc_buf_ensure(s.seed, (size_t)pairs * n * sizeof(float2)))) return rc;
    RcFlowAreaArgs a = pl.seed;
    a.src = (const char*)seed.field; a.src_step = seed.step; a.src_pair_stride = seed.pair_stride;
    a.dst = (float2*)s.seed.p; a.dst_pair_stride = n;
    {
        RcProfScope ps(ctx, s.cur, RC_K_FLOW_SEED, k, (double)pairs * (8. * pl.w * pl.h + 8. * n));
        rc_launch_flow_area_init(a, pairs, s.cur);
    }
    *out = (const float2*)s.seed.p;
    return RC_OK;
}

static RcPyrArgs pyr_args(const rc_ctx* ctx, const RcLevel& L, int k, const uint8_t* src, size_t step, size_t frame_stride, int W0,
                          int H0, const float* kern, float* dst, size_t dst_slot_stride, int dslot0, int nslots, int zstep) {
    RcPyrArgs p;
    memset(&p, 0, sizeof(p));
    p.src = src; p.src_step = step; p.src_frame_stride = frame_stride;
    p.W0 = W0; p.H0 = H0;
    p.dst = dst; p.dst_slot_stride = dst_slot_stride;
    p.dslot0 = dslot0; p.nslots = nslots; p.zstep = zstep;
    p.w = L.w; p.h = L.h; p.scale_x = L.scale_x; p.scale_y = L.scale_y;
    p.ksize = L.ksize; p.kern = kern;
    p.tw = L.pyr_tw; p.th = L.pyr_th; p.reg_wp = L.pyr_reg_w; p.reg_hmax = L.pyr_reg_h;
    p.direct = (ctx->ablate & RC_ABL_PYR_STAGED) != 0;
    p.fixed3 = k == 0 && L.ksize == 3 && !(L.sigma > 0) && L.w == W0 && L.h == H0;
    return p;
}

static int expand_frames(rc_ctx* ctx, RcSlot& s, const uint8_t* d_src, size_t frame_stride, size_t step,
                         int count, int dslot0, int zstep = 1) {
    if (!s.in_ts_push) s.ts_streak = 0;
    RcPlan& pl = s.plan;
    RcPolyArgs qa[RC_MAX_LEVELS];
    RcPyrArgs pa[RC_MAX_LEVELS];
    for (int k = 0; k < pl.nlev; k++) {
        const RcLevel& L = pl.lv[k];
        size_t n = (size_t)L.w * L.h;
        RcPolyArgs& q = qa[k];
        memset(&q, 0, sizeof(q));
        q.RA = (float4*)s.RA[k].p; q.RB = (float*)s.RB[k].p; q.R_slot_stride = n;
        q.slot0 = dslot0; q.nslots = pl.nslots; q.zstep = zstep; q.w = L.w; q.h = L.h; q.pk = pl.pk;
        q.tile_h = ctx->poly_tile_h; q.valu_vertical = !ctx->poly_mfma;
        if (k == 0 && !pl.exact) {
            q.src8 = d_src; q.src8_step = step; q.src8_frame_stride = frame_stride;
            continue;
        }
        q.I = (const float*)s.I[k].p; q.I_slot_stride = n;
        pa[k] = pyr_args(ctx, L, k, d_src, step, frame_stride, pl.w, pl.h, (const float*)s.kern.p + pl.kern_off[k],
                         (float*)s.I[k].p, n, dslot0, pl.nslots, zstep);
    }
    auto npx = [&](int k) { return (double)pl.lv[k].w * pl.lv[k].h; };
    if (pl.exact) {
        for (int k = 0; k < pl.nlev; k++) {
            { RcProfScope ps(ctx, s.cur, RC_K_PYR, k, (double)count * (npx(0) + 4. * npx(k)));
              rc_launch_pyr(pa[k], count, pl.lv[k].pyr_lds, s.cur); }
            RcProfScope ps(ctx, s.cur, RC_K_POLY, k, (double)count * 24. * npx(k));
            rc_launch_exact_polyexp(qa[k], count, s.cur);
        }
        RC_HIP(hipGetLastError());
        return RC_OK;
    }
    const bool merge = ctx->merge_small && count <= 2;
    int npyr = 0;
    if (!merge && ctx->fuse_pyr && pl.nlev >= 2 && rc_polyexp_pyr_ok(qa[0])) {
        auto exact = [&](int k, int f) { return pl.lv[k].w * f == pl.w && pl.lv[k].h * f == pl.h; };
        if (exact(1, 2) && pl.lv[1].ksize == 3) {
            npyr = 1;
            if (pl.nlev >= 3 && exact(2, 4) && pl.lv[2].ksize == 9) npyr = 2;
        }
    }
    if (npyr) {
        RcPolyArgs& q = qa[0];
        q.npyr = npyr;
        double alg = 21. * npx(0), model = 29. * npx(0);
        for (int k = 1; k <= npyr; k++) {
            q.py[k - 1].dst = pa[k].dst; q.py[k - 1].dst_slot_stride = pa[k].dst_slot_stride;
            q.py[k - 1].w = pa[k].w; q.py[k - 1].h = pa[k].h; q.py[k - 1].kern = pa[k].kern;
            alg += 4. * npx(k); model += npx(0) + 4. * npx(k);
        }
        RcProfScope ps(ctx, s.cur, RC_K_POLY, 0, (double)count * alg, (double)count * model);
        rc_launch_polyexp(q, count, s.cur);
    }
    int k_pyr = 1 + npyr;
    if (merge && pl.nlev >= 3 && rc_pyr_pair_ok(pa[1], pa[2])) {
        RcProfScope ps(ctx, s.cur, RC_K_PYR, 1, (double)count * (2. * npx(0) + 4. * (npx(1) + npx(2))));
        rc_launch_pyr_pair(pa[1], pa[2], count, s.cur);
        k_pyr = 3;
    }
    for (int k = k_pyr; k < pl.nlev; k++) {
        RcProfScope ps(ctx, s.cur, RC_K_PYR, k, (double)count * (npx(0) + 4. * npx(k)));
        rc_launch_pyr(pa[k], count, pl.lv[k].pyr_lds, s.cur);
    }
    int k_poly = 0;
    const int nm = pl.nlev < 3 ? pl.nlev : 3;
    if (merge && nm >= 2 && rc_polyexp_multi_ok(qa, nm)) {
        double alg = 21. * npx(0), model = 29. * npx(0);
        for (int k = 1; k < nm; k++) { alg += 24. * npx(k); model += 24. * npx(k); }
        RcProfScope ps(ctx, s.cur, RC_K_POLY, 0, (double)count * alg, (double)count * model);
        rc_launch_polyexp_multi(qa, nm, count, s.cur);
        k_poly = nm;
    }
    if (npyr) k_poly = 1;
    for (int k = k_poly; k < pl.nlev; k++) {
        RcProfScope ps(ctx, s.cur, RC_K_POLY, k, (double)count * (k == 0 ? 21. : 24.) * npx(k),
                       k == 0 ? (double)count * 29. * npx(0) : -1.);
        rc_launch_polyexp(qa[k], count, s.cur);
    }
    RC_HIP(hipGetLastError());
    return RC_OK;
}

static int compute_flows_exact(rc_ctx* ctx, RcSlot& s, int pairs, int slot0, float* d_out, size_t out_pair_stride,
                               size_t out_step, int slot1, int zstep, const RcSeed* seed) {
    RcPlan& pl = s.plan;
    const int iters = pl.prm.iterations;
    const size_t n0 = (size_t)pl.lv[0].w * pl.lv[0].h;
    int rc;
    if ((rc = rc_buf_ensure(s.exM, n0 * 5 * pairs * sizeof(float)))) return rc;
    const size_t n0p = (size_t)pl.lv[0].w * ((pl.lv[0].h + 15) & ~15);
    if ((rc = rc_buf_ensure(s.exV, pl.win.gaussian ? n0 * 5 * pairs * sizeof(float) : n0p * 5 * pairs * sizeof(double)))) return rc;
    if (!pl.win.gaussian && (rc = rc_buf_ensure(s.exG, n0 * 5 * pairs * sizeof(double)))) return rc;
    const float2* seeded = nullptr;
    if (seed && (rc = launch_seed(ctx, s, pairs, *seed, &seeded))) return rc;
    const float2* coarse = nullptr;
    int cw = 0, ch = 0;
    for (int k = pl.nlev - 1; k >= 0; k--) {
        const RcLevel& L = pl.lv[k];
        RcExactArgs a;
        memset(&a, 0, sizeof(a));
        a.RA = (const float4*)s.RA[k].p; a.RB = (const float*)s.RB[k].p; a.n = (size_t)L.w * L.h;
        a.slot0 = slot0; a.slot1 = slot1 >= 0 ? slot1 : (slot0 + 1) % pl.nslots; a.nslots = pl.nslots; a.zstep = zstep;
        a.w = L.w; a.h = L.h; a.win = pl.win; a.plain_scans = (ctx->ablate & RC_ABL_EXACT_PLAIN_SCANS) != 0;
        a.fused_matrices = (ctx->ablate & RC_ABL_EXACT_FUSED_M) != 0;
        a.flow = (float2*)s.FA[k].p; a.M = (float*)s.exM.p; a.V = s.exV.p; a.G = s.exG.p;
        if (coarse) {
            a.fin = coarse; a.fin_pair_stride = (size_t)cw * ch; a.fin_w = cw; a.fin_h = ch;
            a.up_scale_x = 1. / ((double)L.w / cw); a.up_scale_y = 1. / ((double)L.h / ch);
            a.up_mul = (float)(1. / pl.prm.pyr_scale);
        } else if (seeded) {
            a.fin = seeded; a.fin_pair_stride = a.n; a.fin_w = L.w; a.fin_h = L.h;
            a.up_scale_x = a.up_scale_y = 1.; a.up_mul = 1.f;
        }
        const double nb = (double)pairs * a.n;
        { RcProfScope ps(ctx, s.cur, RC_K_ITER, k, 8. * nb + (coarse ? 8. * pairs * cw * ch : seeded ? 8. * nb : 0.));
          rc_launch_exact_flow_init(a, pairs, s.cur); }
        for (int i = 0; i < iters; i++) {
            if (k == 0 && i == iters - 1) { a.out = (char*)d_out; a.out_step = out_step; a.out_pair_stride = out_pair_stride; }
            if (rc_exact_iteration_fused_ok(a)) {
                RcProfScope ps(ctx, s.cur, RC_K_ITER, k, 136. * nb);
                rc_launch_exact_iteration_fused(a, pairs, s.cur);
                continue;
            }
            { RcProfScope ps(ctx, s.cur, RC_K_ITER, k, 68. * nb); rc_launch_exact_matrices(a, pairs, s.cur); }
            { RcProfScope ps(ctx, s.cur, RC_K_ITER, k, (pl.win.gaussian ? 68. : 108.) * nb);
              rc_launch_exact_window_solve(a, pairs, s.cur); }
        }
        if (k == 0 && iters == 0)
            for (int z = 0; z < pairs; z++)
                RC_HIP(hipMemcpy2DAsync((char*)d_out + (size_t)z * out_pair_stride, out_step, a.flow + (size_t)z * a.n,
                                        (size_t)L.w * 8, (size_t)L.w * 8, (size_t)L.h, hipMemcpyDeviceToDevice, s.cur));
        coarse = a.flow;
        cw = L.w; ch = L.h;
    }
    RC_HIP(hipGetLastError());
    return RC_OK;
}

static int compute_flows(rc_ctx* ctx, RcSlot& s, int pairs, int slot0, float* d_out, size_t out_pair_stride,
                         size_t out_step, int slot1 = -1, int zstep = 1, const RcSeed* seed = nullptr) {
    if (!s.in_ts_push) s.ts_streak = 0;
    if (s.plan.exact && !s.plan.win.gaussian)
        return compute_flows_exact(ctx, s, pairs, slot0, d_out, out_pair_stride, out_step, slot1, zstep, seed);
    const bool exact = s.plan.exact != 0;
    RcPlan& pl = s.plan;
    const int iters = pl.prm.iterations;
    const float2* seeded = nullptr;
    if (seed) { int rc = launch_seed(ctx, s, pairs, *seed, &seeded); if (rc) return rc; }
    const float2* coarse = nullptr;
    int cw = 0, ch = 0;
    for (int k = pl.nlev - 1; k >= 0; k--) {
        const RcLevel& L = pl.lv[k];
        size_t n = (size_t)L.w * L.h;
        RcIterArgs a;
        memset(&a, 0, sizeof(a));
        a.RA = (const float4*)s.RA[k].p; a.RB = (const float*)s.RB[k].p; a.R_slot_stride = n;
        a.slot0 = slot0; a.slot1 = slot1 >= 0 ? slot1 : (slot0 + 1) % pl.nslots; a.nslots = pl.nslots; a.zstep = zstep;
        a.w = L.w; a.h = L.h;
        a.win = pl.win;
        a.xcd_remap = ctx->xcd_remap;
        a.ablate = ctx->ablate;
        a.chain = ctx->chain;
        a.chain_min_blocks = ctx->chain_min_blocks;
        const float2* cur_in = nullptr;
        int passes = iters > 0 ? iters : 1;
        int nout = 0;
        for (int i = 0; i < passes;) {
            double in_bytes;
            if (i == 0) {
                if (!coarse && seeded) { a.in_mode = 1; a.fin = seeded; a.fin_pair_stride = n; in_bytes = 8. * n; }
                else if (!coarse) { a.in_mode = 0; a.fin = nullptr; in_bytes = 0; }
                else {
                    a.in_mode = 2; a.fin = coarse; a.fin_pair_stride = (size_t)cw * ch;
                    a.fin_w = cw; a.fin_h = ch;
                    a.up_scale_x = 1. / ((double)L.w / cw);
                    a.up_scale_y = 1. / ((double)L.h / ch);
                    a.up_mul = (float)(1. / pl.prm.pyr_scale);
                    a.up_exact2 = (L.w == 2 * cw && L.h == 2 * ch) ? 1 : 0;
                    in_bytes = 8. * cw * ch;
                }
            } else {
                a.in_mode = 1; a.fin = cur_in; a.fin_pair_stride = n; in_bytes = 8. * n;
            }
            a.solve = iters > 0 ? 1 : 0;
            a.addr32 = n * 16 < (1ull << 32) && (size_t)L.h * (k == 0 ? (out_step > (size_t)L.w * 8 ? out_step : (size_t)L.w * 8) : (size_t)L.w * 8) < (1ull << 32);
            int fuse = (passes - i >= 2 && ctx->fuse_iters && rc_flow_fast::rc_flow_iter_can_fuse2(a)) ? 2 : 1;
            bool last = (i + fuse == passes);
            if (last && k == 0) {
                a.fout = (char*)d_out; a.fout_step = out_step; a.fout_pair_stride = out_pair_stride;
            } else {
                float2* dst = (float2*)((nout & 1) ? s.FB[k].p : s.FA[k].p);
                nout++;
                a.fout = (char*)dst; a.fout_step = (size_t)L.w * 8; a.fout_pair_stride = n * 8;
                cur_in = dst;
            }
            {
                double model = 0;
                if (i == 0) model += 60. * n + (coarse ? 8. * cw * ch : 0.);
                for (int j = i; j < i + fuse; j++) model += (j == passes - 1) ? 28. * n : 80. * n;
                const int r0 = fuse != 2 ? pairs : exact ? rc_flow_exact::rc_flow_iter2_r0_reads(a, pairs) : rc_flow_fast::rc_flow_iter2_r0_reads(a, pairs);
                RcProfScope ps(ctx, s.cur, fuse == 2 ? RC_K_ITER2 : RC_K_ITER, k,
                               (a.solve ? 20. * n * (pairs + r0) : 0.) + (double)pairs * (in_bytes + 8. * n), (double)pairs * model);
                if (exact) {
                    if (fuse == 2) rc_flow_exact::rc_launch_flow_iter2(a, pairs, s.cur);
                    else rc_flow_exact::rc_launch_flow_iter(a, pairs, s.cur);
                } else {
                    if (fuse == 2) rc_flow_fast::rc_launch_flow_iter2(a, pairs, s.cur);
                    else rc_flow_fast::rc_launch_flow_iter(a, pairs, s.cur);
                }
            }
            i += fuse;
        }
        coarse = cur_in;
        cw = L.w; ch = L.h;
    }
    RC_HIP(hipGetLastError());
    return RC_OK;
}

static int pair_check(const char* who, const char* prev_name, const void* prev, size_t prev_step, const char* next_name, const void* next,
                      size_t next_step, const char* flow_name, const void* flow, size_t flow_step, int w, int h) {
    int rc;
    if ((rc = rc_image_check(who, prev_name, prev, prev_step, w, h, 1, 1, RC_ARG_IN))) return rc;
    if ((rc = rc_image_check(who, next_name, next, next_step, w, h, 1, 1, RC_ARG_IN))) return rc;
    return rc_image_check(who, flow_name, flow, flow_step, w, h, 8, 1, RC_ARG_OUT);
}

extern "C" int rcflow_farneback_dev(rc_ctx* ctx, int stream, const uint8_t* d_prev, size_t prev_step,
                                    const uint8_t* d_next, size_t next_step, int w, int h, float* d_flow,
                                    size_t flow_step, const rc_farneback_params* p) {
    RcSlot* s = rc_slot(ctx, stream);
    if (!s) return RC_EINVAL;
    int rc = pair_check(__func__, "d_prev", d_prev, prev_step, "d_next", d_next, next_step, "d_flow", d_flow, flow_step, w, h);
    if (rc) return rc;
    RC_HIP(hipSetDevice(ctx->device));
    if ((rc = ensure_plan(__func__, ctx, *s, w, h, p, ctx->chunk))) return rc;
    s->primed = 0;
    s->batch_primed = 0;
    s->flow_w = s->flow_h = 0;
    s->flow_fresh = 0;
    if ((rc = expand_frames(ctx, *s, d_prev, 0, prev_step, 1, 0))) return rc;
    if ((rc = expand_frames(ctx, *s, d_next, 0, next_step, 1, 1))) return rc;
    const RcSeed seed = {d_flow, flow_step, 0};
    const bool use_seed = (p->flags & RC_FARNEBACK_USE_INITIAL_FLOW) != 0;
    if (use_seed && !seed_layout_ok(__func__, d_flow, flow_step, 0)) return RC_EINVAL;
    return compute_flows(ctx, *s, 1, 0, d_flow, 0, flow_step, -1, 1, use_seed ? &seed : nullptr);
}

extern "C" int rcflow_farneback_u8(rc_ctx* ctx, int stream, const uint8_t* prev, size_t prev_step,
                                   const uint8_t* next, size_t next_step, int w, int h, float* flow,
                                   size_t flow_step, double pyr_scale, int levels, int winsize, int iterations,
                                   int poly_n, double poly_sigma, int flags) {
    RcSlot* s = rc_slot(ctx, stream);
    if (!s) return RC_EINVAL;
    int rc = pair_check(__func__, "prev", prev, prev_step, "next", next, next_step, "flow", flow, flow_step, w, h);
    if (rc) return rc;
    rc_farneback_params p = {pyr_scale, levels, winsize, iterations, poly_n, poly_sigma, flags};
    RC_HIP(hipSetDevice(ctx->device));
    if ((rc = ensure_plan(__func__, ctx, *s, w, h, &p, ctx->chunk))) return rc;
    size_t fb = (size_t)w * h;
    if ((rc = rc_buf_ensure(s->stage_u8, 2 * fb))) return rc;
    if ((rc = rc_buf_ensure(s->stage_flow, fb * 8))) return rc;
    uint8_t* du = (uint8_t*)s->stage_u8.p;
    RC_HIP(hipMemcpy2DAsync(du, w, prev, prev_step, w, h, hipMemcpyHostToDevice, s->cur));
    RC_HIP(hipMemcpy2DAsync(du + fb, w, next, next_step, w, h, hipMemcpyHostToDevice, s->cur));
    if (flags & RC_FARNEBACK_USE_INITIAL_FLOW)
        RC_HIP(hipMemcpy2DAsync(s->stage_flow.p, (size_t)w * 8, flow, flow_step, (size_t)w * 8, h, hipMemcpyHostToDevice, s->cur));
    rc = rcflow_farneback_dev(ctx, stream, du, w, du + fb, w, w, h, (float*)s->stage_flow.p, (size_t)w * 8, &p);
    if (rc) return rc;
    RC_HIP(hipMemcpy2DAsync(flow, flow_step, s->stage_flow.p, (size_t)w * 8, (size_t)w * 8, h,
                            hipMemcpyDeviceToHost, s->cur));
    RC_HIP(hipStreamSynchronize(s->cur));
    return RC_OK;
}

extern "C" int rcflow_stream_reset(rc_ctx* ctx, int stream) {
    RcSlot* s = rc_slot(ctx, stream);
    if (!s) return RC_EINVAL;
    s->primed = 0;
    s->cur_slot = 0;
    s->flow_w = s->flow_h = 0;
    s->flow_fresh = 0;
    return RC_OK;
}

struct RcFrameAux {
    const void* host_src; void* d_dst; size_t bytes;
    hipEvent_t after_upload;
};

static int push_frame_core(const char* who, rc_ctx* ctx, RcSlot* s, const uint8_t* d_frame, size_t step, int w, int h,
                           float* d_flow, size_t flow_step, const rc_farneback_params* p, bool two_streams,
                           const RcFrameAux* up, bool resident) {
    int rc = ensure_plan(who, ctx, *s, w, h, p, ctx->chunk);
    if (rc) return rc;
    s->batch_primed = 0;
    auto upload_on = [&](hipStream_t st) -> int {
        if (!up) return RC_OK;
        RC_HIP(hipMemcpyAsync(up->d_dst, up->host_src, up->bytes, hipMemcpyHostToDevice, st));
        RC_HIP(hipEventRecord(up->after_upload, st));
        return RC_OK;
    };
    if (!s->primed) {
        if ((rc = upload_on(s->cur))) return rc;
        if ((rc = expand_frames(ctx, *s, d_frame, 0, step, 1, 0))) return rc;
        s->primed = 1;
        s->cur_slot = 0;
        s->flow_fresh = 0;
        return 1;
    }
    if ((rc = rc_image_check(who, "d_flow", d_flow, flow_step, w, h, 8, 1, RC_ARG_OUT))) return rc;
    const RcSeed seed_desc = {d_flow, flow_step, 0};
    const bool use_seed = (p->flags & RC_FARNEBACK_USE_INITIAL_FLOW) && (!resident || s->flow_fresh);
    if (use_seed && !seed_layout_ok(who, d_flow, flow_step, 0)) return RC_EINVAL;
    const RcSeed* seed = use_seed ? &seed_desc : nullptr;
    s->flow_fresh = 0;
    const int nxt = (s->cur_slot + 1) % s->plan.nslots;
    if (two_streams && !ctx->prof_on && s->plan.nslots >= 4) {
        if (!s->aux) RC_HIP(hipStreamCreateWithFlags(&s->aux, hipStreamNonBlocking));
        for (auto& e : s->flow_done) if (!e) { RC_HIP(hipEventCreateWithFlags(&e, hipEventDisableTiming)); RC_HIP(hipEventRecord(e, s->cur)); }
        hipStream_t main_stream = s->cur;
        const int older = s->flow_done_i;
        if (s->ts_streak == 0) {
            hipEvent_t& joined = s->fev[s->fev_i];
            s->fev_i = (s->fev_i + 1) % 8;
            if (!joined) RC_HIP(hipEventCreateWithFlags(&joined, hipEventDisableTiming));
            RC_HIP(hipEventRecord(joined, main_stream));
            RC_HIP(hipStreamWaitEvent(s->aux, joined, 0));
        } else {
            RC_HIP(hipStreamWaitEvent(s->aux, s->flow_done[older], 0));
        }
        hipEvent_t& expanded = s->fev[s->fev_i];
        s->fev_i = (s->fev_i + 1) % 8;
        if (!expanded) RC_HIP(hipEventCreateWithFlags(&expanded, hipEventDisableTiming));
        if ((rc = upload_on(s->aux))) return rc;
        s->in_ts_push = true;
        s->cur = s->aux;
        rc = expand_frames(ctx, *s, d_frame, 0, step, 1, nxt);
        s->cur = main_stream;
        if (rc) { s->in_ts_push = false; return rc; }
        RC_HIP(hipEventRecord(expanded, s->aux));
        RC_HIP(hipStreamWaitEvent(main_stream, expanded, 0));
        rc = compute_flows(ctx, *s, 1, s->cur_slot, d_flow, 0, flow_step, -1, 1, seed);
        s->in_ts_push = false;
        if (rc) return rc;
        RC_HIP(hipEventRecord(s->flow_done[older], main_stream));
        s->flow_done_i = older ^ 1;
        s->ts_streak++;
        s->cur_slot = nxt;
        return RC_OK;
    }
    if ((rc = upload_on(s->cur))) return rc;
    if ((rc = expand_frames(ctx, *s, d_frame, 0, step, 1, nxt))) return rc;
    if ((rc = compute_flows(ctx, *s, 1, s->cur_slot, d_flow, 0, flow_step, -1, 1, seed))) return rc;
    s->cur_slot = nxt;
    return RC_OK;
}

extern "C" int rcflow_push_frame_dev(rc_ctx* ctx, int stream, const uint8_t* d_frame, size_t step, int w, int h,
                                     float* d_flow, size_t flow_step, const rc_farneback_params* p) {
    RcSlot* s = rc_slot(ctx, stream);
    if (!s) return RC_EINVAL;
    if (int rc = rc_image_check(__func__, "d_frame", d_frame, step, w, h, 1, 1, RC_ARG_IN)) return rc;
    RC_HIP(hipSetDevice(ctx->device));
    return push_frame_core(__func__, ctx, s, d_frame, step, w, h, d_flow, flow_step, p, ctx->frame_overlap >= 2, nullptr, false);
}

static int frame_staging_next(const char* who, rc_ctx* ctx, RcSlot* s, int w, int h, int* idx) {
    if (w <= 0 || h <= 0) { rc_set_error("%s: an empty size %d x %d", who, w, h); return RC_EINVAL; }
    if (int rc = rc_fits_context(who, ctx, w, h)) return rc;
    RC_HIP(hipSetDevice(ctx->device));
    const size_t fb = (size_t)w * h;
    if (s->pin_bytes < fb) {
        RC_HIP(hipStreamSynchronize(s->cur));
        for (int i = 0; i < 2; i++) {
            if (s->pin[i]) (void)hipHostFree(s->pin[i]);
            s->pin[i] = nullptr;
            if (hipHostMalloc(&s->pin[i], fb, hipHostMallocDefault) != hipSuccess) { rc_set_error("%s: hipHostMalloc(%zu) failed", who, fb); s->pin_bytes = 0; return RC_ENOMEM; }
            if (!s->pin_free[i]) RC_HIP(hipEventCreateWithFlags(&s->pin_free[i], hipEventDisableTiming));
            RC_HIP(hipEventRecord(s->pin_free[i], s->cur));
        }
        s->pin_bytes = fb;
    }
    int rc;
    if ((rc = rc_buf_ensure(s->stage_u8, 2 * fb))) return rc;
    if ((rc = rc_buf_ensure(s->stage_flow, fb * 8))) return rc;
    RC_HIP(hipEventSynchronize(s->pin_free[s->pin_i]));
    *idx = s->pin_i;
    return RC_OK;
}

static int push_staged_frame(const char* who, rc_ctx* ctx, RcSlot* s, int i, int w, int h, const rc_farneback_params* p) {
    const size_t fb = (size_t)w * h;
    uint8_t* d_frame = (uint8_t*)s->stage_u8.p + (size_t)i * fb;
    s->pin_i = i ^ 1;
    s->pin_acq = -1;
    RcFrameAux up = {s->pin[i], d_frame, fb, s->pin_free[i]};
    const int rc = push_frame_core(who, ctx, s, d_frame, w, w, h, (float*)s->stage_flow.p, (size_t)w * 8, p, ctx->frame_overlap >= 1, &up, true);
    if (rc == RC_OK) { s->flow_w = w; s->flow_h = h; s->flow_fresh = 1; }
    else if (rc == 1) { s->flow_w = s->flow_h = 0; }
    return rc;
}

extern "C" int rcflow_push_frame_u8(rc_ctx* ctx, int stream, const uint8_t* frame, size_t step, int w, int h,
                                    const rc_farneback_params* p) {
    RcSlot* s = rc_slot(ctx, stream);
    if (!s) return RC_EINVAL;
    int i, rc;
    if ((rc = rc_image_check(__func__, "frame", frame, step, w, h, 1, 1, RC_ARG_IN))) return rc;
    if ((rc = frame_staging_next(__func__, ctx, s, w, h, &i))) return rc;
    uint8_t* dst = (uint8_t*)s->pin[i];
    if (step == (size_t)w) memcpy(dst, frame, (size_t)w * h);
    else for (int y = 0; y < h; y++) memcpy(dst + (size_t)y * w, frame + (size_t)y * step, w);
    return push_staged_frame(__func__, ctx, s, i, w, h, p);
}

extern "C" int rcflow_frame_buffer_acquire(rc_ctx* ctx, int stream, int w, int h, uint8_t** host_frame, size_t* step) {
    RcSlot* s = rc_slot(ctx, stream);
    if (!s) return RC_EINVAL;
    int i, rc;
    if ((rc = rc_ptr_check(__func__, "host_frame", host_frame))) return rc;
    if ((rc = frame_staging_next(__func__, ctx, s, w, h, &i))) return rc;
    s->pin_acq = i; s->pin_w = w; s->pin_h = h;
    *host_frame = (uint8_t*)s->pin[i];
    if (step) *step = (size_t)w;
    return RC_OK;
}
extern "C" int rcflow_push_frame_acquired(rc_ctx* ctx, int stream, const rc_farneback_params* p) {
    RcSlot* s = rc_slot(ctx, stream);
    if (!s) return RC_EINVAL;
    if (s->pin_acq < 0 || s->pin_acq != s->pin_i) { rc_set_error("%s: no frame buffer acquired (rcflow_frame_buffer_acquire) since the last push", __func__); return RC_ESTATE; }
    RC_HIP(hipSetDevice(ctx->device));
    return push_staged_frame(__func__, ctx, s, s->pin_acq, s->pin_w, s->pin_h, p);
}

extern "C" int rcflow_stream_flow_ptr(rc_ctx* ctx, int stream, float** d_flow, int* w, int* h) {
    RcSlot* s = rc_slot(ctx, stream);
    if (!s) return RC_EINVAL;
    if (int rc = rc_ptr_check(__func__, "d_flow", d_flow)) return rc;
    if (!s->flow_w) { rc_set_error("%s: no flow field yet: the stream has only been primed", __func__); return RC_ESTATE; }
    *d_flow = (float*)s->stage_flow.p;
    if (w) *w = s->flow_w;
    if (h) *h = s->flow_h;
    return RC_OK;
}

extern "C" int rcflow_stream_flow_read(rc_ctx* ctx, int stream, float* flow, size_t flow_step) {
    RcSlot* s = rc_slot(ctx, stream);
    if (!s) return RC_EINVAL;
    int rc;
    if ((rc = rc_ptr_check(__func__, "flow", flow))) return rc;
    if (!s->flow_w) { rc_set_error("%s: no flow field yet: the stream has only been primed", __func__); return RC_ESTATE; }
    if (flow_step < (size_t)s->flow_w * 8) { rc_set_error("%s: flow_step %zu below the %zu bytes of a row of flow", __func__, flow_step, (size_t)s->flow_w * 8); return RC_EINVAL; }
    RC_HIP(hipSetDevice(ctx->device));
    RC_HIP(hipMemcpy2DAsync(flow, flow_step, s->stage_flow.p, (size_t)s->flow_w * 8, (size_t)s->flow_w * 8, s->flow_h,
                            hipMemcpyDeviceToHost, s->cur));
    RC_HIP(hipStreamSynchronize(s->cur));
    return RC_OK;
}

extern "C" int rcflow_push_clip_dev(rc_ctx* ctx, int stream, const uint8_t* d_frames, size_t frame_stride, size_t step,
                                    int nframes, int w, int h, float* d_flows, size_t flow_frame_stride,
                                    size_t flow_step, const rc_farneback_params* p) {
    RcSlot* s = rc_slot(ctx, stream);
    if (!s) return RC_EINVAL;
    if (nframes < 1) { rc_set_error("%s: nframes %d (>= 1)", __func__, nframes); return RC_EINVAL; }
// ... 456 lines not shown
```

Baseline: 20070.

## Drive interior flow-iteration tiles from host-built per-thread offset tables

Adds a per-level, per-form table of precomputed per-thread offsets (window load offsets, LDS handles, exchange-row offsets, row index), built on the host at plan time and uploaded to the device. Interior tiles now run a dedicated table-driven body that reads these offsets instead of recomputing index arithmetic, while the generic body loses its INTERIOR template specialisation. The aim is to cut integer address math and register pressure in the hot iteration kernel. In exchange it adds extra global loads of the table records and restricts the supported tile shapes to the forms listed in the table.

```diff
diff --git a/ripcurrents_amd/csrc/flow_iter_kernels.hip b/ripcurrents_amd/csrc/flow_iter_kernels.hip
--- a/ripcurrents_amd/csrc/flow_iter_kernels.hip
+++ b/ripcurrents_amd/csrc/flow_iter_kernels.hip
@@ -773,48 +773,78 @@
         : "v"(V[0]), "v"(V[1]), "v"(V[2]), "v"(V[3]), "v"(V[4]));
 }
 
+template <int GAUSS_, int NIT, int MW>
+__device__ __forceinline__ void rc_rr_flows_at(const float (&m)[NIT][5], const float* XU, const float* XD,
+                                               const RcWindow& win, float2 (&f)[NIT]) {
+    float up[5], dn[5];
+#pragma unroll
+    for (int c = 0; c < 5; c++) {
+        up[c] = XU[(5 + c) * MW];
+        dn[c] = XD[c * MW];
+    }
+    float V[NIT][5];
+#pragma unroll
+    for (int q = 0; q < NIT; q++)
+#pragma unroll
+        for (int c = 0; c < 5; c++) {
+            float u = q > 0 ? m[q - 1][c] : up[c], d = q < NIT - 1 ? m[q + 1][c] : dn[c];
+            if (GAUSS_) V[q][c] = m[q][c] * win.k[0] + (d + u) * win.k[1];
+            else V[q][c] = m[q][c] + (d + u);
+        }
+#pragma unroll
+    for (int q = 0; q < NIT; q++) {
+        float g[5];
+        if (GAUSS_) {
+            float lr[5];
+            rc_hpair_dpp(lr, V[q]);
+#pragma unroll
+            for (int c = 0; c < 5; c++) g[c] = V[q][c] * win.k[0] + win.k[1] * lr[c];
+        } else {
+            rc_hsum3_dpp(g, V[q]);
+        }
+        f[q] = rc_solve3(g, GAUSS_ ? 1e-3f : (float)win.box_eps);
+    }
+}
+
 template <int GAUSS_, int NIT, int MW, int NG>
 __device__ __forceinline__ void rc_rr_flows(const float (&m)[NIT][5], const float* XR, int grp, int x,
                                             const RcWindow& win, float2 (&f)[NIT]) {
     const int gu = max(grp - 1, 0), gd = min(grp + 1, NG - 1);
     const int bu = (int)__umul24((unsigned)gu, 10u * MW) + x, bd = (int)__umul24((unsigned)gd, 10u * MW) + x;
-    float up[5], dn[5];
+    rc_rr_flows_at<GAUSS_, NIT, MW>(m, XR + bu, XR + bd, win, f);
+}
+
+template <int NIT, int MW>
+__device__ __forceinline__ void rc_rr_exchange_at(const float (&m)[NIT][5], float* XB) {
 #pragma unroll
     for (int c = 0; c < 5; c++) {
-        up[c] = XR[bu + (5 + c) * MW];
-        dn[c] = XR[bd + c * MW];
-    }
-    float V[NIT][5];
-#pragma unroll
-    for (int q = 0; q < NIT; q++)
-#pragma unroll
-        for (int c = 0; c < 5; c++) {
-            float u = q > 0 ? m[q - 1][c] : up[c], d = q < NIT - 1 ? m[q + 1][c] : dn[c];
-            if (GAUSS_) V[q][c] = m[q][c] * win.k[0] + (d + u) * win.k[1];
-            else V[q][c] = m[q][c] + (d + u);
-        }
-#pragma unroll
-    for (int q = 0; q < NIT; q++) {
-        float g[5];
-        if (GAUSS_) {
-            float lr[5];
-            rc_hpair_dpp(lr, V[q]);
-#pragma unroll
-            for (int c = 0; c < 5; c++) g[c] = V[q][c] * win.k[0] + win.k[1] * lr[c];
-        } else {
-            rc_hsum3_dpp(g, V[q]);
-        }
-        f[q] = rc_solve3(g, GAUSS_ ? 1e-3f : (float)win.box_eps);
+        XB[c * MW] = m[0][c];
+        XB[(5 + c) * MW] = m[NIT - 1][c];
     }
 }
 
 template <int NIT, int MW>
 __device__ __forceinline__ void rc_rr_exchange(const float (&m)[NIT][5], float* XR, int grp, int x) {
-    const int b = (int)__umul24((unsigned)grp, 10u * MW) + x;
-#pragma unroll
-    for (int c = 0; c < 5; c++) {
-        XR[b + c * MW] = m[0][c];
-        XR[b + (5 + c) * MW] = m[NIT - 1][c];
+    rc_rr_exchange_at<NIT, MW>(m, XR + ((int)__umul24((unsigned)grp, 10u * MW) + x));
+}
+
+template <int NIT>
+__device__ __forceinline__ void rc_rr_up2_rows(const float2 (&t0)[NIT / 2 + 2], const float2 (&t1)[NIT / 2 + 2], float ax, float up_mul,
+                                               float (&dx)[NIT], float (&dy)[NIT]) {
+    constexpr int NR = NIT / 2 + 2;
+    const float a0 = 1.f - ax, a1 = ax;
+    float hx[NR], hy[NR];
+#pragma unroll
+    for (int j = 0; j < NR; j++) {
+        hx[j] = t0[j].x * a0 + t1[j].x * a1;
+        hy[j] = t0[j].y * a0 + t1[j].y * a1;
+    }
+#pragma unroll
+    for (int q = 0; q < NIT; q++) {
+        const int j0 = (q + 1) >> 1;
+        const float b1 = (q & 1) ? 0.25f : 0.75f, b0 = 1.f - b1;
+        dx[q] = (hx[j0] * b0 + hx[j0 + 1] * b1) * up_mul;
+        dy[q] = (hy[j0] * b0 + hy[j0 + 1] * b1) * up_mul;
     }
 }
 
@@ -831,28 +861,18 @@
         for (int q = 0; q < NIT; q++) d[q] = INTERIOR ? fin[(unsigned)(gys[q] * w + gxo)] : fin[(size_t)gys[q] * w + gxo];
 #pragma unroll
         for (int q = 0; q < NIT; q++) { dx[q] = d[q].x; dy[q] = d[q].y; }
-    } else if ((NIT % 2 == 0) && a.up_exact2 && (INTERIOR || (ty0 - 2 >= 0 && ty0 - 2 + MH <= h))) {
+    } else if (!INTERIOR && (NIT % 2 == 0) && a.up_exact2 && ty0 - 2 >= 0 && ty0 - 2 + MH <= h) {
         constexpr int NR = NIT / 2 + 2;
         int sx = (gxo - 1) >> 1;
         float ax = (gxo & 1) ? 0.25f : 0.75f;
-        if (!INTERIOR) {
-            if (sx < 0) { ax = 0.f; sx = 0; }
-            if (sx >= a.fin_w - 1) { ax = 0.f; sx = a.fin_w - 1; }
-        }
+        if (sx < 0) { ax = 0.f; sx = 0; }
+        if (sx >= a.fin_w - 1) { ax = 0.f; sx = a.fin_w - 1; }
         const int sx1 = min(sx + 1, a.fin_w - 1);
         const int rb = (gys[0] - 1) >> 1;
         float2 t0[NR], t1[NR];
         typedef float rc_f4a8 __attribute__((ext_vector_type(4), aligned(8)));
-        const bool cols_plain = INTERIOR || (tx0 - 2 >= 1 && tx0 - 2 + MW <= w && ((tx0 - 2 + MW - 2) >> 1) + 1 <= a.fin_w - 1);
-        if (INTERIOR) {
-            unsigned co = (unsigned)(__mul24(rb, a.fin_w) + sx);
-#pragma unroll
-            for (int j = 0; j < NR; j++) {
-                const rc_f4a8 v = *(const rc_f4a8*)(fin + co);
-                t0[j] = make_float2(v.x, v.y); t1[j] = make_float2(v.z, v.w);
-                co += (unsigned)a.fin_w;
-            }
-        } else if (cols_plain) {
+        const bool cols_plain = tx0 - 2 >= 1 && tx0 - 2 + MW <= w && ((tx0 - 2 + MW - 2) >> 1) + 1 <= a.fin_w - 1;
+        if (cols_plain) {
 #pragma unroll
             for (int j = 0; j < NR; j++) {
                 const float2* S = fin + (size_t)rc_clampi(rb + j, 0, a.fin_h - 1) * a.fin_w;
@@ -866,20 +886,7 @@
                 t0[j] = S[sx]; t1[j] = S[sx1];
             }
         }
-        const float a0 = 1.f - ax, a1 = ax;
-        float hx[NR], hy[NR];
-#pragma unroll
-        for (int j = 0; j < NR; j++) {
-            hx[j] = t0[j].x * a0 + t1[j].x * a1;
-            hy[j] = t0[j].y * a0 + t1[j].y * a1;
-        }
-#pragma unroll
-        for (int q = 0; q < NIT; q++) {
-            const int j0 = (q + 1) >> 1;
-            const float b1 = (q & 1) ? 0.25f : 0.75f, b0 = 1.f - b1;
-            dx[q] = (hx[j0] * b0 + hx[j0 + 1] * b1) * a.up_mul;
-            dy[q] = (hy[j0] * b0 + hy[j0 + 1] * b1) * a.up_mul;
-        }
+        rc_rr_up2_rows<NIT>(t0, t1, ax, a.up_mul, dx, dy);
     } else {
         float2 p00[NIT], p01[NIT], p10[NIT], p11[NIT];
         float ax, ay[NIT];
@@ -934,7 +941,7 @@
     asm volatile("s_mov_b32 m0, %2\n\ts_nop 0\n\tglobal_load_lds_dword %0, %1" ::"v"(voff), "s"(base), "s"(lds_wave_addr) : "memory");
 }
 
-template <bool INTERIOR, int NT, int WP, int WN, int NWL>
+template <int NT, int WP, int WN, int NWL>
 __device__ __forceinline__ void rc_rrc_issue_window(const float4* __restrict__ RA1, const float* __restrict__ RB1,
                                                     uint32_t lds_a, uint32_t lds_b, int tid, int ox, int oy, int w, int h) {
     constexpr int QY = NT / WP, QX = NT % WP;
@@ -945,7 +952,7 @@
 #pragma unroll
     for (int q = 0; q < NWL; q++) {
         bool ok = (q + 1) * NT <= WN || tid + q * NT < WN;
-        if (!INTERIOR) ok = ok && (unsigned)(ox + wx) < (unsigned)w && (unsigned)(oy + wy) < (unsigned)h;
+        ok = ok && (unsigned)(ox + wx) < (unsigned)w && (unsigned)(oy + wy) < (unsigned)h;
         const unsigned p = ok ? (unsigned)off : 0u;
         if (q * NT + wave_base < WN) {
             rc_glds16_s(RA1, p << 4, lds_a + (uint32_t)(q * NT + wave_base) * 16u);
@@ -956,56 +963,75 @@
     }
 }
 
-template <bool INTERIOR, int NIT, int WW, int WH, int WP>
+template <int NT, int WN, int NWL>
+__device__ __forceinline__ void rc_rrc_issue_window_tab(const float4* __restrict__ WA, const float* __restrict__ WB,
+                                                        uint32_t lds_a, uint32_t lds_b, int tid, const uint32_t (&wo)[NWL]) {
+    const int wave_base = __builtin_amdgcn_readfirstlane(tid & ~63);
+#pragma unroll
+    for (int q = 0; q < NWL; q++) {
+        if (q * NT + wave_base < WN) {
+            rc_glds16_s(WA, wo[q], lds_a + (uint32_t)(q * NT + wave_base) * 16u);
+            rc_glds4_s(WB, wo[q] >> 2, lds_b + (uint32_t)(q * NT + wave_base) * 4u);
+        }
+    }
+}
+
+template <int NIT, int WW, int WH, int WP>
 __device__ __forceinline__ void rc_rr_matrices(float (&m)[NIT][5], const float4 (&A0)[NIT], const float (&B0)[NIT],
                                                const float (&dx)[NIT], const float (&dy)[NIT], const float4* LA,
                                                const float* LB, int ox, int oy, const float4* __restrict__ RA1,
                                                const float* __restrict__ RB1, int gxo, const int (&gys)[NIT], int w, int h) {
-    if constexpr (!INTERIOR) {
+#pragma unroll
+    for (int q = 0; q < NIT; q++) {
+        RcGather g;
+        rc_gather_window<WW, WH, WP>(g, LA, LB, ox, oy, RA1, RB1, gxo, gys[q], dx[q], dy[q], w, h);
+        RcM5 v = rc_matrices_reg(A0[q], B0[q], g, dx[q], dy[q], gxo, gys[q], w, h, true);
+        m[q][0] = v.m0; m[q][1] = v.m1; m[q][2] = v.m2; m[q][3] = v.m3; m[q][4] = v.m4;
+    }
+}
+
+template <int NIT, int WW, int WH, int WP, int MW>
+__device__ __forceinline__ void rc_rr_matrices_tab(float (&m)[NIT][5], const float4 (&A0)[NIT], const float (&B0)[NIT],
+                                                   const float (&dx)[NIT], const float (&dy)[NIT], const float4* LA,
+                                                   const float* LB, int ox, int oy, const float4* __restrict__ RA1,
+                                                   const float* __restrict__ RB1, float fgx, const float (&fgy)[NIT],
+                                                   int tid, int tx0, int ty0, int w, int h) {
+    unsigned far = 0;
+#pragma unroll
+    for (int q = 0; q < NIT; q++) {
+        RcGather g;
+        const float fx = fgx + dx[q], fy = fgy[q] + dy[q];
+        const float flx = floorf(fx), fly = floorf(fy);
+        const int x1 = (int)flx, y1 = (int)fly;
+        g.fx = fx - flx;
+        g.fy = fy - fly;
+        g.inside = true;
+        const int wx = x1 - ox, wy = y1 - oy;
+        const bool in_win = (unsigned)wx < (unsigned)(WW - 1) && (unsigned)wy < (unsigned)(WH - 1);
+        far |= in_win ? 0u : 1u << q;
+        const unsigned i = in_win ? __umul24((unsigned)wy, (unsigned)WP) + (unsigned)wx : 0u;
+        const float4* pa = (const float4*)((const char*)LA + (i << 4));
+        const float* pb = (const float*)((const char*)LB + (i << 2));
+        g.q00 = pa[0]; g.q01 = pa[1]; g.q10 = pa[WP]; g.q11 = pa[WP + 1];
+        g.e00 = pb[0]; g.e01 = pb[1]; g.e10 = pb[WP]; g.e11 = pb[WP + 1];
+        RcM5 v = rc_matrices_reg(A0[q], B0[q], g, dx[q], dy[q], 0, 0, w, h, false);
+        m[q][0] = v.m0; m[q][1] = v.m1; m[q][2] = v.m2; m[q][3] = v.m3; m[q][4] = v.m4;
+    }
+    if (__builtin_expect(far != 0, 0)) {
+        const int gxo = tx0 - 2 + (tid & (MW - 1)), gy0 = ty0 - 2 + tid / MW * NIT;
 #pragma unroll
         for (int q = 0; q < NIT; q++) {
-            RcGather g;
-            rc_gather_window<WW, WH, WP>(g, LA, LB, ox, oy, RA1, RB1, gxo, gys[q], dx[q], dy[q], w, h);
-            RcM5 v = rc_matrices_reg(A0[q], B0[q], g, dx[q], dy[q], gxo, gys[q], w, h, true);
-            m[q][0] = v.m0; m[q][1] = v.m1; m[q][2] = v.m2; m[q][3] = v.m3; m[q][4] = v.m4;
-        }
-    } else {
-        unsigned far = 0;
-#pragma unroll
-        for (int q = 0; q < NIT; q++) {
-            RcGather g;
-            const float fx = gxo + dx[q], fy = gys[q] + dy[q];
-            const float flx = floorf(fx), fly = floorf(fy);
-            const int x1 = (int)flx, y1 = (int)fly;
-            g.fx = fx - flx;
-            g.fy = fy - fly;
-            g.inside = true;
-            const int wx = x1 - ox, wy = y1 - oy;
-            const bool in_win = (unsigned)wx < (unsigned)(WW - 1) && (unsigned)wy < (unsigned)(WH - 1);
-            far |= in_win ? 0u : 1u << q;
-            const unsigned i = in_win ? __umul24((unsigned)wy, (unsigned)WP) + (unsigned)wx : 0u;
-            const float4* pa = (const float4*)((const char*)LA + (i << 4));
-            const float* pb = (const float*)((const char*)LB + (i << 2));
-            g.q00 = pa[0]; g.q01 = pa[1]; g.q10 = pa[WP]; g.q11 = pa[WP + 1];
-            g.e00 = pb[0]; g.e01 = pb[1]; g.e10 = pb[WP]; g.e11 = pb[WP + 1];
-            RcM5 v = rc_matrices_reg(A0[q], B0[q], g, dx[q], dy[q], gxo, gys[q], w, h, false);
-            m[q][0] = v.m0; m[q][1] = v.m1; m[q][2] = v.m2; m[q][3] = v.m3; m[q][4] = v.m4;
-        }
-        if (__builtin_expect(far != 0, 0)) {
-#pragma unroll
-            for (int q = 0; q < NIT; q++) {
-                if (far >> q & 1) {
-                    RcGather g;
-                    rc_gather_issue(g, RA1, RB1, gxo, gys[q], dx[q], dy[q], w, h);
-                    RcM5 v = rc_matrices_reg(A0[q], B0[q], g, dx[q], dy[q], gxo, gys[q], w, h, false);
-                    m[q][0] = v.m0; m[q][1] = v.m1; m[q][2] = v.m2; m[q][3] = v.m3; m[q][4] = v.m4;
-                }
-            }
-        }
-    }
-}
-
-template <bool INTERIOR, int IN_MODE, int GAUSS_, int NIT, int D, int MW, int NG>
+            if (far >> q & 1) {
+                RcGather g;
+                rc_gather_issue(g, RA1, RB1, gxo, gy0 + q, dx[q], dy[q], w, h);
+                RcM5 v = rc_matrices_reg(A0[q], B0[q], g, dx[q], dy[q], gxo, gy0 + q, w, h, false);
+                m[q][0] = v.m0; m[q][1] = v.m1; m[q][2] = v.m2; m[q][3] = v.m3; m[q][4] = v.m4;
+            }
+        }
+    }
+}
+
+template <int IN_MODE, int GAUSS_, int NIT, int D, int MW, int NG>
 __device__ __forceinline__ void rc_rrc_body(const RcIterArgs& a, const int zb, const int ze, float* smf, const uint32_t lds0, const int tx0, const int ty0) {
     constexpr int NT = NG * MW, MH = NG * NIT;
     constexpr int WW = MW + 2 * D, WH = MH + 2 * D, WP = WW, WN = WP * WH, NWL = (WN + NT - 1) / NT;
@@ -1022,10 +1048,10 @@
 #define RC_RRC_COORDS(tid_)                                                         \
     const int x = (tid_) & (MW - 1), grp = (tid_) / MW, ly0 = grp * NIT;            \
     const int px = tx0 - 2 + x;                                                     \
-    const int gxo = INTERIOR ? px : rc_clampi(px, 0, w - 1);                        \
+    const int gxo = rc_clampi(px, 0, w - 1);                                       \
     int gys[NIT];                                                                   \
     _Pragma("unroll") for (int q = 0; q < NIT; q++)                                 \
-        gys[q] = INTERIOR ? ty0 - 2 + ly0 + q : rc_clampi(ty0 - 2 + ly0 + q, 0, h - 1);
+        gys[q] = rc_clampi(ty0 - 2 + ly0 + q, 0, h - 1);
 
     float4 A0[NIT];
     float B0[NIT];
@@ -1035,14 +1061,14 @@
         RC_RRC_COORDS(tid)
         const size_t s0 = (size_t)((a.slot0 + zb * a.zstep) % a.nslots) * a.R_slot_stride;
         const size_t s1 = (size_t)((a.slot1 + zb * a.zstep) % a.nslots) * a.R_slot_stride;
-        rc_rrc_issue_window<INTERIOR, NT, WP, WN, NWL>(a.RA + s1, a.RB + s1, lds_a, lds_b, tid, ox, oy, w, h);
+        rc_rrc_issue_window<NT, WP, WN, NWL>(a.RA + s1, a.RB + s1, lds_a, lds_b, tid, ox, oy, w, h);
 #pragma unroll
         for (int q = 0; q < NIT; q++) {
             const unsigned p0 = (unsigned)(gys[q] * w + gxo);
             A0[q] = (a.RA + s0)[p0];
             B0[q] = (a.RB + s0)[p0];
         }
-        rc_rr_flow_in<IN_MODE, NIT, MW, MH, INTERIOR>(a, a.fin + (size_t)zb * a.fin_pair_stride, tx0, ty0, gxo, gys, dx, dy);
+        rc_rr_flow_in<IN_MODE, NIT, MW, MH>(a, a.fin + (size_t)zb * a.fin_pair_stride, tx0, ty0, gxo, gys, dx, dy);
     }
 
     for (int z = zb; z < ze; z++) {
@@ -1056,7 +1082,7 @@
         rc_all_barrier();
 
         float m[NIT][5];
-        rc_rr_matrices<INTERIOR, NIT, WW, WH, WP>(m, A0, B0, dx, dy, LA, LB, ox, oy, RA1, RB1, gxo, gys, w, h);
+        rc_rr_matrices<NIT, WW, WH, WP>(m, A0, B0, dx, dy, LA, LB, ox, oy, RA1, RB1, gxo, gys, w, h);
         rc_rr_exchange<NIT, MW>(m, XR, grp, x);
         rc_lds_barrier();
 
@@ -1066,7 +1092,7 @@
             float f1x[NIT], f1y[NIT];
 #pragma unroll
             for (int q = 0; q < NIT; q++) { f1x[q] = f1[q].x; f1y[q] = f1[q].y; }
-            rc_rr_matrices<INTERIOR, NIT, WW, WH, WP>(m, A0, B0, f1x, f1y, LA, LB, ox, oy, RA1, RB1, gxo, gys, w, h);
+            rc_rr_matrices<NIT, WW, WH, WP>(m, A0, B0, f1x, f1y, LA, LB, ox, oy, RA1, RB1, gxo, gys, w, h);
         }
         if (more) {
 #pragma unroll
@@ -1077,20 +1103,18 @@
             }
         }
         rc_lds_barrier();
-        if constexpr (!INTERIOR) {
-#pragma unroll
-            for (int q = 0; q < NIT; q++)
-#pragma unroll
-                for (int c = 0; c < 5; c++) Ms[c * PLANE + (ly0 + q) * MP + x] = m[q][c];
-            rc_lds_barrier();
-#pragma unroll
-            for (int q = 0; q < NIT; q++) {
-                const int py = ty0 - 2 + ly0 + q;
-                if ((unsigned)px >= (unsigned)w || (unsigned)py >= (unsigned)h) {
-                    const int cx = gxo - (tx0 - 2), cy = gys[q] - (ty0 - 2);
-#pragma unroll
-                    for (int c = 0; c < 5; c++) m[q][c] = Ms[c * PLANE + cy * MP + cx];
-                }
+#pragma unroll
+        for (int q = 0; q < NIT; q++)
+#pragma unroll
+            for (int c = 0; c < 5; c++) Ms[c * PLANE + (ly0 + q) * MP + x] = m[q][c];
+        rc_lds_barrier();
+#pragma unroll
+        for (int q = 0; q < NIT; q++) {
+            const int py = ty0 - 2 + ly0 + q;
+            if ((unsigned)px >= (unsigned)w || (unsigned)py >= (unsigned)h) {
+                const int cx = gxo - (tx0 - 2), cy = gys[q] - (ty0 - 2);
+#pragma unroll
+                for (int c = 0; c < 5; c++) m[q][c] = Ms[c * PLANE + cy * MP + cx];
             }
         }
         rc_rr_exchange<NIT, MW>(m, XR, grp, x);
@@ -1098,26 +1122,156 @@
 
         if (more) {
             const size_t n1 = (size_t)((a.slot1 + (z + 1) * a.zstep) % a.nslots) * a.R_slot_stride;
-            rc_rrc_issue_window<INTERIOR, NT, WP, WN, NWL>(a.RA + n1, a.RB + n1, lds_a, lds_b, tid, ox, oy, w, h);
+            rc_rrc_issue_window<NT, WP, WN, NWL>(a.RA + n1, a.RB + n1, lds_a, lds_b, tid, ox, oy, w, h);
         }
 
         {
             char* fout = a.fout + (size_t)z * a.fout_pair_stride;
             float2 f2[NIT];
             rc_rr_flows<GAUSS_, NIT, MW, NG>(m, XR, grp, x, a.win, f2);
-            if (x >= 2 && x < MW - 2 && (INTERIOR || px < w)) {
+            if (x >= 2 && x < MW - 2 && px < w) {
                 unsigned so = (unsigned)(ty0 - 2 + ly0) * (unsigned)a.fout_step + (unsigned)px * 8u;
 #pragma unroll
                 for (int q = 0; q < NIT; q++) {
                     const int ly = ly0 + q, py = ty0 - 2 + ly;
-                    if (ly >= 2 && ly < MH - 2 && (INTERIOR || py < h)) *(float2*)(fout + so) = f2[q];
+                    if (ly >= 2 && ly < MH - 2 && py < h) *(float2*)(fout + so) = f2[q];
                     so += (unsigned)a.fout_step;
                 }
             }
         }
-        if (more) rc_rr_flow_in<IN_MODE, NIT, MW, MH, INTERIOR>(a, a.fin + (size_t)(z + 1) * a.fin_pair_stride, tx0, ty0, gxo, gys, dx, dy);
+        if (more) rc_rr_flow_in<IN_MODE, NIT, MW, MH>(a, a.fin + (size_t)(z + 1) * a.fin_pair_stride, tx0, ty0, gxo, gys, dx, dy);
     }
 #undef RC_RRC_COORDS
+}
+
+template <int IN_MODE, int NIT, int MW, int MH>
+__device__ __forceinline__ void rc_rrc_flow_in_tab(const RcIterArgs& a, const float2* __restrict__ fin, int tx0, int ty0, int tid,
+                                                   float (&dx)[NIT], float (&dy)[NIT]) {
+    if constexpr (IN_MODE == 2 && NIT % 2 == 0) {
+        if (a.up_exact2) {
+            constexpr int NR = NIT / 2 + 2;
+            typedef float rc_f4a8 __attribute__((ext_vector_type(4), aligned(8)));
+            const float2* cb = fin + (unsigned)((((ty0 - 2) >> 1) - 1) * a.fin_w + ((tx0 - 2) >> 1) - 1);
+            const unsigned x = (unsigned)tid & (MW - 1), ly0 = (unsigned)tid / MW * NIT;
+            const unsigned co = __umul24((ly0 + 1) >> 1, (unsigned)a.fin_w) + ((x + 1) >> 1);
+            float2 t0[NR], t1[NR];
+#pragma unroll
+            for (int j = 0; j < NR; j++) {
+                const rc_f4a8 v = *(const rc_f4a8*)(cb + (unsigned)(j * a.fin_w) + co);
+                t0[j] = make_float2(v.x, v.y); t1[j] = make_float2(v.z, v.w);
+            }
+            rc_rr_up2_rows<NIT>(t0, t1, (x & 1) ? 0.25f : 0.75f, a.up_mul, dx, dy);
+            return;
+        }
+    }
+    const int gxo = tx0 - 2 + (tid & (MW - 1));
+    int gys[NIT];
+#pragma unroll
+    for (int q = 0; q < NIT; q++) gys[q] = ty0 - 2 + tid / MW * NIT + q;
+    rc_rr_flow_in<IN_MODE, NIT, MW, MH, true>(a, fin, tx0, ty0, gxo, gys, dx, dy);
+}
+
+template <int IN_MODE, int GAUSS_, int NIT, int D, int MW, int NG>
+__device__ __forceinline__ void rc_rrc_body_tab(const RcIterArgs& a, const int zb, const int ze, float* smf, const uint32_t lds0, const int tx0, const int ty0) {
+    constexpr int NT = NG * MW, MH = NG * NIT;
+    constexpr int WW = MW + 2 * D, WH = MH + 2 * D, WP = WW, WN = WP * WH, NWL = (WN + NT - 1) / NT;
+    constexpr int WNP = (WN + 63) & ~63;
+    static_assert(NWL <= RC_RRC_NWL, "the record holds every slice of the window");
+    float4* LA = (float4*)smf;
+    float* LB = smf + 4 * WNP;
+    float* XR = LB + WNP;
+    const uint32_t lds_a = lds0, lds_b = lds0 + 16u * WNP;
+    const int w = a.w, h = a.h;
+    const int ox = tx0 - 2 - D, oy = ty0 - 2 - D;
+    const unsigned worg = (unsigned)(oy * w + ox);
+
+    float4 A0[NIT];
+    float B0[NIT];
+    float dx[NIT], dy[NIT];
+    float fgx, fgy[NIT];
+    unsigned xb, xu, xd, hand;
+    uint32_t wo[NWL];
+    {
+        const int tid = threadIdx.x;
+        const RcRrcRec* r = a.rrc_tab + tid;
+        const int x = tid & (MW - 1);
+        const unsigned ly0 = (unsigned)tid / MW * NIT;
+        const float fly0 = r->fly0;
+        xb = r->xr_b; xu = r->xr_u; xd = r->xr_d; hand = r->hand;
+#pragma unroll
+        for (int q = 0; q < NWL; q++) wo[q] = r->win[q];
+        asm volatile("" ::"v"(fly0), "v"(xb), "v"(xu), "v"(xd), "v"(hand));
+#pragma unroll
+        for (int q = 0; q < NWL; q++) asm volatile("" ::"v"(wo[q]));
+        fgx = (float)(tx0 - 2 + x);
+#pragma unroll
+        for (int q = 0; q < NIT; q++) fgy[q] = (float)(ty0 - 2 + q) + fly0;
+        const size_t s0 = (size_t)((a.slot0 + zb * a.zstep) % a.nslots) * a.R_slot_stride;
+        const size_t s1 = (size_t)((a.slot1 + zb * a.zstep) % a.nslots) * a.R_slot_stride;
+        rc_rrc_issue_window_tab<NT, WN, NWL>(a.RA + s1 + worg, a.RB + s1 + worg, lds_a, lds_b, tid, wo);
+        const unsigned p0 = (unsigned)((ty0 - 2) * w + tx0 - 2) + __umul24(ly0, (unsigned)w) + (unsigned)x;
+#pragma unroll
+        for (int q = 0; q < NIT; q++) {
+            A0[q] = (a.RA + s0)[p0 + (unsigned)(q * w)];
+            B0[q] = (a.RB + s0)[p0 + (unsigned)(q * w)];
+        }
+        rc_rrc_flow_in_tab<IN_MODE, NIT, MW, MH>(a, a.fin + (size_t)zb * a.fin_pair_stride, tx0, ty0, tid, dx, dy);
+    }
+
+    for (int z = zb; z < ze; z++) {
+        const size_t s1 = (size_t)((a.slot1 + z * a.zstep) % a.nslots) * a.R_slot_stride;
+        const float4* __restrict__ RA1 = a.RA + s1;
+        const float* __restrict__ RB1 = a.RB + s1;
+        const bool more = z + 1 < ze;
+        int tid = threadIdx.x;
+        asm volatile("" : "+v"(tid));
+        rc_all_barrier();
+
+        float m[NIT][5];
+        rc_rr_matrices_tab<NIT, WW, WH, WP, MW>(m, A0, B0, dx, dy, LA, LB, ox, oy, RA1, RB1, fgx, fgy, tid, tx0, ty0, w, h);
+        rc_rr_exchange_at<NIT, MW>(m, (float*)((char*)XR + xb));
+        rc_lds_barrier();
+
+        {
+            float2 f1[NIT];
+            rc_rr_flows_at<GAUSS_, NIT, MW>(m, (const float*)((const char*)XR + xu), (const float*)((const char*)XR + xd), a.win, f1);
+            float f1x[NIT], f1y[NIT];
+#pragma unroll
+            for (int q = 0; q < NIT; q++) { f1x[q] = f1[q].x; f1y[q] = f1[q].y; }
+            rc_rr_matrices_tab<NIT, WW, WH, WP, MW>(m, A0, B0, f1x, f1y, LA, LB, ox, oy, RA1, RB1, fgx, fgy, tid, tx0, ty0, w, h);
+        }
+        if (more) {
+            const float4* ha = (const float4*)((const char*)LA + (hand << 2));
+            const float* hb = (const float*)((const char*)LB + hand);
+#pragma unroll
+            for (int q = 0; q < NIT; q++) {
+                A0[q] = ha[q * WP];
+                B0[q] = hb[q * WP];
+            }
+        }
+        rc_lds_barrier();
+        rc_rr_exchange_at<NIT, MW>(m, (float*)((char*)XR + xb));
+        rc_lds_barrier();
+
+        if (more) {
+            const size_t n1 = (size_t)((a.slot1 + (z + 1) * a.zstep) % a.nslots) * a.R_slot_stride;
+            rc_rrc_issue_window_tab<NT, WN, NWL>(a.RA + n1 + worg, a.RB + n1 + worg, lds_a, lds_b, tid, wo);
+        }
+
+        {
+            char* fout = a.fout + (size_t)z * a.fout_pair_stride + (size_t)(ty0 - 2) * a.fout_step + (size_t)(tx0 - 2) * 8;
+            float2 f2[NIT];
+            rc_rr_flows_at<GAUSS_, NIT, MW>(m, (const float*)((const char*)XR + xu), (const float*)((const char*)XR + xd), a.win, f2);
+            const unsigned x = (unsigned)tid & (MW - 1), ly0 = (unsigned)tid / MW * NIT;
+            if (x - 2 < MW - 4) {
+                const unsigned so = ly0 * (unsigned)a.fout_step + x * 8u;
+#pragma unroll
+                for (int q = 0; q < NIT; q++)
+                    if (ly0 + q - 2 < MH - 4) *(float2*)(fout + (size_t)q * a.fout_step + so) = f2[q];
+            }
+        }
+        if (more) rc_rrc_flow_in_tab<IN_MODE, NIT, MW, MH>(a, a.fin + (size_t)(z + 1) * a.fin_pair_stride, tx0, ty0, tid, dx, dy);
+    }
 }
 
 template <int IN_MODE, int GAUSS_, int NIT, int D, int MINB, int MW, int NG>
@@ -1129,8 +1283,14 @@
     const int tx0 = (t % a.tiles_x) * TW, ty0 = (t / a.tiles_x) * TH;
     const bool interior = tx0 - 2 >= 5 && tx0 - 2 + MW <= a.w - 5 && ty0 - 2 >= 5 && ty0 - 2 + MH <= a.h - 5;
     const uint32_t lds0 = (uint32_t)(uintptr_t)(__attribute__((address_space(3))) void*)smf;
-    if (interior) rc_rrc_body<true, IN_MODE, GAUSS_, NIT, D, MW, NG>(a, zb, ze, smf, lds0, tx0, ty0);
-    else rc_rrc_body<false, IN_MODE, GAUSS_, NIT, D, MW, NG>(a, zb, ze, smf, lds0, tx0, ty0);
+    if (interior && a.rrc_tab) rc_rrc_body_tab<IN_MODE, GAUSS_, NIT, D, MW, NG>(a, zb, ze, smf, lds0, tx0, ty0);
+    else rc_rrc_body<IN_MODE, GAUSS_, NIT, D, MW, NG>(a, zb, ze, smf, lds0, tx0, ty0);
+}
+
+constexpr int rc_rrc_form(int nit, int d) {
+    for (int f = 0; f < RC_RRC_FORMS; f++)
+        if (kRcRrcForms[f][0] == nit && kRcRrcForms[f][1] == d) return f;
+    return -1;
 }
 
 template <int IN_MODE, int G, int NIT, int D, int MINB, int MW = 32, int NG = 8>
@@ -1138,6 +1298,8 @@
     constexpr int MH = NG * NIT, TW = MW - 4, TH = MH - 4;
     a.tw = TW; a.th = TH;
     a.tiles_x = (a.w + TW - 1) / TW; a.tiles_y = (a.h + TH - 1) / TH;
+    static_assert(MW == RC_RRC_MW && NG == RC_RRC_NG && rc_rrc_form(NIT, D) >= 0, "rc_plan.h lists the forms the thread tables are built for");
+    if (a.rrc_tab) a.rrc_tab += rc_rrc_form(NIT, D) * NG * MW;
     constexpr int WN = (MW + 2 * D) * (MH + 2 * D), WNP = (WN + 63) & ~63;
     const size_t lds = sizeof(float) * (5 * WNP + NG * 2 * 5 * MW);
     RC_ALLOW_LDS((k_flow_iter2_rrc<IN_MODE, G, NIT, D, MINB, MW, NG>), lds);
diff --git a/ripcurrents_amd/csrc/rc_common.h b/ripcurrents_amd/csrc/rc_common.h
--- a/ripcurrents_amd/csrc/rc_common.h
+++ b/ripcurrents_amd/csrc/rc_common.h
@@ -112,6 +112,7 @@
     int addr32;
     int chain_min_blocks;
     int chain;
+    const RcRrcRec* rrc_tab;
     RcWindow win;
 };
 
diff --git a/ripcurrents_amd/csrc/rc_host.h b/ripcurrents_amd/csrc/rc_host.h
--- a/ripcurrents_amd/csrc/rc_host.h
+++ b/ripcurrents_amd/csrc/rc_host.h
@@ -335,6 +335,7 @@
     RcBuf kern;
     RcBuf I[RC_MAX_LEVELS], RA[RC_MAX_LEVELS], RB[RC_MAX_LEVELS];
     RcBuf FA[RC_MAX_LEVELS], FB[RC_MAX_LEVELS];
+    RcBuf rrc_tab;
     RcBuf stage_u8, stage_flow, stage_f32[4];
     RcBuf exM, exV, exG;
     void* pin[2] = {nullptr, nullptr};
diff --git a/ripcurrents_amd/csrc/rc_plan.cpp b/ripcurrents_amd/csrc/rc_plan.cpp
--- a/ripcurrents_amd/csrc/rc_plan.cpp
+++ b/ripcurrents_amd/csrc/rc_plan.cpp
@@ -193,6 +193,29 @@
     }
 }
 
+int rc_plan_rrc_table(int w, int MW, int NG, int NIT, int D, RcRrcRec* rec) {
+    if (w <= 0 || MW < 8 || (MW & (MW - 1)) || NG < 1 || NIT < 1 || NIT > 4 || D < 0 || !rec) return RC_EINVAL;
+    const int NT = NG * MW, MH = NG * NIT, WP = MW + 2 * D, WH = MH + 2 * D, WN = WP * WH;
+    if ((WN + NT - 1) / NT > RC_RRC_NWL) return RC_EINVAL;
+    if (((unsigned long long)(WH - 1) * (unsigned)w + WP) * 16ull >= (1ull << 32)) return RC_EINVAL;
+    for (int tid = 0; tid < NT; tid++) {
+        RcRrcRec& r = rec[tid];
+        memset(&r, 0, sizeof(r));
+        const int x = tid % MW, grp = tid / MW, ly0 = grp * NIT;
+        for (int q = 0; q < RC_RRC_NWL; q++) {
+            const int idx = tid + q * NT;
+            if (idx < WN) r.win[q] = (uint32_t)(((size_t)(idx / WP) * w + idx % WP) * 16);
+        }
+        r.hand = (uint32_t)(((ly0 + D) * WP + x + D) * 4);
+        const int gu = grp > 0 ? grp - 1 : 0, gd = grp < NG - 1 ? grp + 1 : NG - 1;
+        r.xr_b = (uint32_t)((10 * MW * grp + x) * 4);
+        r.xr_u = (uint32_t)((10 * MW * gu + x) * 4);
+        r.xr_d = (uint32_t)((10 * MW * gd + x) * 4);
+        r.fly0 = (float)ly0;
+    }
+    return RC_OK;
+}
+
 int rc_plan_params_valid(const rc_farneback_params* p) {
     if (!p) return 0;
     if (!(p->pyr_scale > 0 && p->pyr_scale < 1)) return 0;
diff --git a/ripcurrents_amd/csrc/rc_plan.h b/ripcurrents_amd/csrc/rc_plan.h
--- a/ripcurrents_amd/csrc/rc_plan.h
+++ b/ripcurrents_amd/csrc/rc_plan.h
@@ -1,6 +1,7 @@
 #pragma once
 
 #include <stddef.h>
+#include <stdint.h>
 
 #include "../../include/rcflow.h"
 
@@ -41,6 +42,20 @@
     int gaussian;
 };
 
+#define RC_RRC_NWL 6
+struct alignas(16) RcRrcRec {
+    uint32_t win[RC_RRC_NWL];
+    uint32_t hand;
+    uint32_t xr_b, xr_u, xr_d;
+    float fly0;
+    uint32_t pad;
+};
+#define RC_RRC_FORMS 3
+#define RC_RRC_MW 32
+#define RC_RRC_NG 8
+static constexpr int kRcRrcForms[RC_RRC_FORMS][2] = {{4, 3}, {2, 4}, {3, 4}};
+int rc_plan_rrc_table(int w, int MW, int NG, int NIT, int D, RcRrcRec* rec);
+
 int rc_plan_params_valid(const rc_farneback_params* p);
 int rc_plan_crop_levels(int w, int h, double pyr_scale, int levels);
 void rc_plan_level_geom(int w, int h, double pyr_scale, int k, RcLevel& L);
diff --git a/ripcurrents_amd/csrc/rcflow_api.hip b/ripcurrents_amd/csrc/rcflow_api.hip
--- a/ripcurrents_amd/csrc/rcflow_api.hip
+++ b/ripcurrents_amd/csrc/rcflow_api.hip
@@ -224,6 +224,7 @@
         rc_buf_free(s.I[k]); rc_buf_free(s.RA[k]); rc_buf_free(s.RB[k]);
         rc_buf_free(s.FA[k]); rc_buf_free(s.FB[k]);
     }
+    rc_buf_free(s.rrc_tab);
     rc_graph_drop(s.batch_graph);
     rc_buf_free(s.stage_u8); rc_buf_free(s.stage_flow); rc_buf_free(s.lk); rc_buf_free(s.fit_ws); rc_buf_free(s.area_tab);
     rc_buf_free(s.seed); rc_buf_free(s.seed_tab);
@@ -349,6 +350,15 @@
     memcpy(xga, pk.xga, (n + 1) * sizeof(float));
     memcpy(xgb, pk.xgb, (n + 1) * sizeof(float));
     *kdch = pk.kdch;
+    return RC_OK;
+}
+extern "C" int rcflow_debug_plan_rrc_table(int w, int MW, int NG, int NIT, int D, uint32_t* words, int cap_words) {
+    if (int rc = rc_ptr_check(__func__, "words", words)) return rc;
+    static_assert(sizeof(RcRrcRec) == 48, "a record is three 16-byte words");
+    if (w <= 0 || MW <= 0 || NG <= 0 || MW > 1024 || NG > 1024 || cap_words < NG * MW * 12) { rc_set_error("%s: w %d, MW %d, NG %d or cap_words %d (12 per thread)", __func__, w, MW, NG, cap_words); return RC_EINVAL; }
+    std::vector<RcRrcRec> rec((size_t)NG * MW);
+    if (rc_plan_rrc_table(w, MW, NG, NIT, D, rec.data())) { rc_set_error("%s: the form (MW %d, NG %d, NIT %d, D %d) at width %d does not fit the record", __func__, MW, NG, NIT, D, w); return RC_EINVAL; }
+    memcpy(words, rec.data(), rec.size() * sizeof(RcRrcRec));
     return RC_OK;
 }
 extern "C" int rcflow_debug_plan_pyr_kernel(int ksize, double sigma, float* taps) {
@@ -485,6 +495,18 @@
         if ((rc = rc_buf_ensure(s.FA[k], n * chunk * sizeof(float2)))) return rc;
         if ((rc = rc_buf_ensure(s.FB[k], n * chunk * sizeof(float2)))) return rc;
     }
+    {
+        constexpr int NT = RC_RRC_NG * RC_RRC_MW;
+        std::vector<RcRrcRec> th((size_t)(L + 1) * RC_RRC_FORMS * NT);
+        for (int k = 0; k <= L; k++)
+            for (int f = 0; f < RC_RRC_FORMS; f++)
+                if (rc_plan_rrc_table(pl.lv[k].w, RC_RRC_MW, RC_RRC_NG, kRcRrcForms[f][0], kRcRrcForms[f][1], th.data() + ((size_t)k * RC_RRC_FORMS + f) * NT)) {
+                    rc_set_error("%s: scale %d is too wide for the flow kernel's thread table", who, k);
+                    return RC_ESIZE;
+                }
+        if ((rc = rc_buf_ensure(s.rrc_tab, th.size() * sizeof(RcRrcRec)))) return rc;
+        RC_HIP(hipMemcpy(s.rrc_tab.p, th.data(), th.size() * sizeof(RcRrcRec), hipMemcpyHostToDevice));
+    }
     memset(&pl.seed, 0, sizeof(pl.seed));
     if (p->flags & RC_FARNEBACK_USE_INITIAL_FLOW) {
         if ((rc = rc_flow_area_prepare(s.seed_tab, w, h, pl.lv[L].w, pl.lv[L].h, pl.seed))) return rc;
@@ -703,6 +725,7 @@
         a.ablate = ctx->ablate;
         a.chain = ctx->chain;
         a.chain_min_blocks = ctx->chain_min_blocks;
+        a.rrc_tab = (const RcRrcRec*)s.rrc_tab.p + (size_t)k * RC_RRC_FORMS * RC_RRC_NG * RC_RRC_MW;
         const float2* cur_in = nullptr;
         int passes = iters > 0 ? iters : 1;
         int nout = 0;
```

After: 20160 (median of 6 runs). No clear change (+0.5%).
